# jcmgray/cotengra

Measured on AMD Instinct MI355X. Metric: contracted FLOP/s (whole node), Sycamore n53 m20 sliced amplitude, higher is better.
Workload: dtype complex64; 1 GPU; Sycamore n53 m20 amplitude, sliced tree, one slice per step per GPU; network=examples/benchmarks/sycamore_n53_m20_s0_e0_pABCDCDAB.json, tree=sycamore_m20_native.json, width_log2=32, parallelism=slice-parallel x1, 1 RCCL reduce, arithmetic=fp16x2 stem pairs and long tiled steps + fp32 MFMA

## Files before the change

cotengra_amd/csrc/ctg_common.h:

```cpp
#pragma once

#include <hip/hip_runtime.h>
#include <cstdlib>
#include <type_traits>
#include <stdint.h>

namespace ctg {

inline bool env_on(const char* name) {
    const char* v = getenv(name);
    return v != nullptr && v[0] != '\0' && !(v[0] == '0' && v[1] == '\0');
}
inline int env_state(const char* name) { return getenv(name) == nullptr ? -1 : (env_on(name) ? 1 : 0); }

inline hipError_t lds_opt_in(const void* kern, int bytes, unsigned long long* done) {
    int dev = 0;
    hipError_t e = hipGetDevice(&dev);
    if (e != hipSuccess) return e;
    const unsigned long long bit = 1ull << (dev & 63);
    if (__atomic_load_n(done, __ATOMIC_ACQUIRE) & bit) return hipSuccess;
    e = hipFuncSetAttribute(kern, hipFuncAttributeMaxDynamicSharedMemorySize, bytes);
    if (e != hipSuccess) {
        (void)hipGetLastError();
        return e;
// ... 353 lines not shown
inline hipError_t for_each_z(const StepArgs& p, F launch_one) {
    if (p.nz <= 1) return launch_one(p);
    for (int z = 0; z < p.nz; ++z) {
        StepArgs q = p;
        q.z0 = p.z0 + z;
        q.nz = 1;
        const hipError_t e = launch_one(q);
        if (e != hipSuccess) return e;
    }
    return hipSuccess;
}

template <typename F>
inline hipError_t for_each_z_chunk(const StepArgs& p, int64_t fit, F launch_chunk) {
    if (fit < 1) fit = 1;
    for (int64_t z = 0; z < p.nz; z += fit) {
        StepArgs q = p;
        q.z0 = p.z0 + (int32_t)z;
        q.nz = (int32_t)(p.nz - z < fit ? p.nz - z : fit);
        const hipError_t e = launch_chunk(q);
        if (e != hipSuccess) return e;
    }
    return hipSuccess;
}


hipError_t launch_pair_valu(int dtype, const StepArgs& p, void* scratch, int64_t scratch_bytes,
                            hipStream_t stream);
struct ValuGroupItem {
    StepArgs p;
    int64_t col_tiles, n_tiles;
    int32_t tn_shift;
    uint32_t block_begin, n_blocks;
};
constexpr int64_t kValuGroupMaxTiles = 4096;
bool valu_thread_per_output(const StepArgs& p);
void pair_valu_name(int dtype, const StepArgs& p, int64_t scratch_bytes, char* buf, size_t n);
uint32_t valu_group_fill(const StepArgs& p, ValuGroupItem* it, uint32_t block_begin);
hipError_t launch_pair_valu_group(int dtype, const ValuGroupItem* d_items, int n_items, uint32_t blocks,
                                  int nz, hipStream_t stream);
hipError_t launch_pair_mfma(int dtype, const StepArgs& p, const MfmaHints& h, void* scratch,
                            int64_t scratch_bytes, hipStream_t stream);
constexpr int64_t kPickKredMinK = 1 << 15, kPickKredMaxM = 512;
inline bool pick_route_kred(int64_t M, int64_t K) { return K >= kPickKredMinK && M <= kPickKredMaxM; }
hipError_t launch_pair_pick(int dtype, const StepArgs& p, int vec, void* scratch, int64_t scratch_bytes,
                            hipStream_t stream);
void pair_pick_name(int dtype, const StepArgs& p, int vec, int64_t scratch_bytes, char* buf, size_t n);
constexpr int64_t kPickRowsMfmaMinRowLo = 32, kPickRowsMfmaMinN = 8, kPickRowsMfmaMinK = 8;
inline bool pick_rows_route_mfma(int64_t row_lo, int64_t K, int64_t N, int dtype) {
    return dtype == 2 && row_lo >= kPickRowsMfmaMinRowLo && N >= kPickRowsMfmaMinN && K >= kPickRowsMfmaMinK;
}
hipError_t launch_pair_pick_rows(int dtype, const StepArgs& p, int vec, int b_fixed, hipStream_t stream);
void pair_pick_rows_name(int dtype, const StepArgs& p, int vec, int b_fixed, char* buf, size_t n);
struct FastGroupItem {
    StepArgs p;
    MfmaHints h;
    int64_t tiles_m, tiles_n;
    uint32_t block_begin, n_blocks;
};
constexpr int64_t kFastGroupMaxTiles = 128;
int fast_group_key(const StepArgs& p, const MfmaHints& h);
uint32_t fast_group_fill(const StepArgs& p, const MfmaHints& h, FastGroupItem* it, uint32_t block_begin);
hipError_t launch_pair_mfma_fast_group(int key, const FastGroupItem* d_items, int n_items, uint32_t blocks,
                                       int nz, hipStream_t stream);
bool rowwise_ok(const StepArgs& p);
void pair_mfma_c64_name(const StepArgs& p, const MfmaHints& h, int64_t scratch_bytes, char* buf, size_t n);
int64_t fast_lane_table_bytes();
hipError_t launch_fast_lane_consts(const StepArgs& p, const MfmaHints& h, void* out, hipStream_t stream);
hipError_t launch_pair_mfma_c128(const StepArgs& p, int flags, hipStream_t stream);
void pair_mfma_c128_name(const StepArgs& p, char* buf, size_t n);
hipError_t launch_pair_mfma_real(int dtype, const StepArgs& p, int flags, hipStream_t stream);
void pair_mfma_real_name(int dtype, const StepArgs& p, int flags, char* buf, size_t n);
bool stem2_supported(const StemArgs& p);
bool stem3_supported(const StemArgs& p);
hipError_t launch_stem2(const StemArgs& p, hipStream_t stream);
void stem2_kernel_name(const StemArgs& p, char* buf, size_t n);
bool stem2h_supported(const StemArgs& p);
bool stem2h_uses_h2(const StemArgs& p);
bool stem2_uses_bf3(const StemArgs& p);
hipError_t launch_stem2h(const StemArgs& p, hipStream_t stream);
void stem2h_kernel_name(const StemArgs& p, char* buf, size_t n);
int stem2_last_paired();
int stem2h_last_paired();

hipError_t launch_single(int dtype, const StepArgs& p, hipStream_t stream);
bool pair_bf16x3_on(const StepArgs& p);
hipError_t launch_accum(int dtype, const StepArgs& p, const StripState* st, void* wide, const double* inscale, int leaf,
                        hipStream_t stream);
struct AccumGroupItem {
    StepArgs p;
    void* wide;
    int32_t leaf;
    uint32_t block_begin, n_blocks;
};
constexpr int64_t kAccumGroupMaxBlocks = 1 << 16;
uint32_t accum_group_fill(const StepArgs& p, void* wide, int leaf, AccumGroupItem* it, uint32_t block_begin);
hipError_t launch_accum_group(int dtype, const AccumGroupItem* d_items, int n_items, uint32_t blocks, int nz,
                              const double* inscale, hipStream_t stream);
hipError_t launch_prescale_inputs(int dtype, void* inputs, const int64_t* offs, const int64_t* sizes, int64_t n_inputs,
                                  int* shift_total, double* inscale, hipStream_t stream);
hipError_t launch_narrow(int dtype, void* result, const void* wide, int64_t n, hipStream_t stream);
hipError_t launch_widen(int dtype, void* wide, const void* result, int64_t n, hipStream_t stream);

hipError_t launch_maxabs(int dtype, const void* x, int64_t n, double* fac, hipStream_t stream);
hipError_t launch_strip_prepare(const double* fac, const int32_t* counted, int64_t n_steps,
                                int64_t root_step, int check_zero, StripState* st, const double* inscale, hipStream_t stream);
hipError_t launch_rescale(int dtype, void* result, int64_t n, const StripState* st, hipStream_t stream);

struct SliceMeta {
    int64_t n_leaves;
    int64_t n_sliced;
    const int64_t* sizes;
    const int64_t* fixed;
    const int64_t* strides;
    double* fac;
    const int32_t* fac_zero;
    int64_t n_fac;
    float* smax;
    const int32_t* smax_zero;
    int64_t n_smax;
};
hipError_t launch_prologue(const SliceMeta& m, int64_t* state, int64_t* soff, int64_t sid,
                           hipStream_t stream, int nz = 1, int64_t stride = 1, const int64_t* ids = nullptr);
hipError_t launch_set_state(int64_t* state, int64_t next, int64_t stride, hipStream_t stream);

}
```

cotengra_amd/csrc/ctg_exec_state.h:

```cpp
#pragma once

#include <string>
#include <vector>

#include "../../include/ctg_hip.h"
#include "ctg_common.h"
#include "ctg_lds.h"

struct ctg_plan {
    int dtype = 0;
    int64_t n_inputs = 0;
    std::vector<int64_t> input_sizes, input_offsets;
    int64_t inputs_elems = 0, arena_elems = 0, result_elems = 0;
    int64_t n_steps = 0;
    std::vector<int64_t> steps;
    std::vector<int64_t> tables;
    int64_t n_sliced = 0;
    std::vector<int64_t> slice_sizes, slice_fixed, slice_strides;
    std::vector<int64_t> slice_group;
    bool has_groups = false;
    int64_t nslices = 1;
    std::vector<int64_t> max_soff;
};

struct ctg_exec {
    const ctg_plan* plan = nullptr;
    int device = 0;
    hipStream_t stream = nullptr;
    char* d_inputs = nullptr;
    char* d_arena = nullptr;
    char* d_result = nullptr;
    bool owns_result = false;
    char* d_wide = nullptr;
    int64_t* d_in_tab = nullptr;
    double* d_inscale = nullptr;
    int64_t* d_tables = nullptr;
    int64_t* d_misc = nullptr;
    int64_t* d_state = nullptr;
    int64_t* d_zero = nullptr;
    int64_t* d_soff = nullptr;
    void* d_scratch = nullptr;
    ctg::SliceMeta meta{};
    std::vector<ctg::StepArgs> args;
    std::vector<ctg::StemArgs> stem_args;
    int stem_bf16x3 = 1;
    int stem_arith = 2;
    float* d_stem_max = nullptr;
    int32_t* d_smax_zero = nullptr;
    float* smax_slot(int bank, int64_t s, int64_t z) const {
        return d_stem_max + (((int64_t)bank * plan_steps + s) * (batch > 1 ? batch : 1) + z) * ctg::kMaxSub;
    }
    ctg::SliceMeta meta_resetting(int which) const {
        ctg::SliceMeta m = meta;
        if (m.smax) m.smax_zero = d_smax_zero + (int64_t)which * m.n_smax;
        return m;
    }
    int64_t plan_steps = 0;
    std::vector<char> rec_wanted;
    std::vector<char> wave_member;
    std::vector<char> stem_paired_ran;
    std::vector<char> stem_h2_ran;
    std::vector<ctg::MfmaHints> hints;
    std::vector<ctg::MfmaHints> hints_b;
    uint16_t* d_ord_b = nullptr;
    char* d_lane_b = nullptr;
    uint16_t* d_ord = nullptr;
    char* d_lane = nullptr;
    int batch = 1;
    int group_d = 0;
    int64_t* d_batch_ids = nullptr;
    int64_t* h_ids = nullptr;
    size_t h_ids_cap = 0;
    hipEvent_t ev_ids = nullptr;
    int batch_nominal = 1;
    int64_t scratch_total = 0;
    struct Issue {
        int64_t step;
        int cls;
        int32_t item0, n;
        uint32_t blocks;
        bool shared = false;
    };
    std::vector<Issue> issue;
    std::vector<Issue> issue_reuse;
    std::vector<int32_t> lds_comp_of;
    int lds_first[2] = {0, 0}, lds_count[2] = {0, 0}, lds_bytes[2] = {0, 0};
    std::vector<std::vector<ctg::LdsForm>> lds_forms;
    ctg::LdsCompDev* d_lds_comps = nullptr;
    char* d_lds_blob = nullptr;
    ctg::ValuGroupItem* d_group_items = nullptr;
    ctg::AccumGroupItem* d_accum_items = nullptr;
    std::vector<char> accum_member;
    ctg::FastGroupItem* d_fast_items = nullptr;
    std::vector<hipEvent_t> events;
    hipStream_t gstream = nullptr;
    hipGraphExec_t gexec = nullptr;
    hipEvent_t ev_in = nullptr, ev_out = nullptr;
    bool warm = false;
    bool soff_static = false;
    bool graph_off = false;
    int strip = 0, check_zero = 0;
    double* d_fac = nullptr;
    int32_t* d_counted = nullptr;
    int32_t* d_fac_zero = nullptr;
    std::vector<char> invariant;
    bool invariants_ready = false;
    std::vector<char> grouped;
    int64_t group_key = -1;
    ctg::StripState* d_strip = nullptr;
    int64_t root_step = -1;
    void* d_sample_blocks = nullptr;
    void* d_sample_io = nullptr;
    int64_t sample_blocks_bytes = 0, sample_io_bytes = 0;
    double sample_last[4] = {0, 0, 0, 0};
    float sample_pass_ms[2] = {0, 0};
    bool sample_last_valid = false;
    hipEvent_t sample_ev[3] = {nullptr, nullptr, nullptr};
    void* d_range = nullptr;
    int64_t range_bytes = 0;
    void* d_reduce = nullptr;
    int64_t reduce_bytes = 0;
};


inline int64_t ctg_item_size(int dtype) {
    static const int64_t k[4] = {4, 8, 8, 16};
    return k[dtype];
}

extern "C" __attribute__((visibility("hidden"))) void ctg_set_error_(const char* msg);

namespace ctg {
hipError_t launch_maxabs_f32(const void* base, const int64_t* soff, int64_t z, int64_t zs, int64_t zstride, int64_t n,
                             float* out, hipStream_t stream, int nz = 1, int out_zs = 0);
}

namespace ctg {
constexpr int64_t kRangeMaxBlocks = 2048;
constexpr int64_t kRangeMaxComponents = 1ll << 40;
int64_t range_blocks(int64_t n);
int64_t range_partial_bytes(int64_t blocks);
hipError_t launch_range_hist(const void* x, int64_t n, void* partials, int64_t blocks, int64_t* row, double* sumsq,
// ... 24 lines not shown
```

cotengra_amd/csrc/ctg_runtime.hip:

```cpp
#include <algorithm>
#include <cstdarg>
#include <cmath>
#include <cstdio>
#include <cstdlib>
#include <cstring>
#include <string>
#include <vector>

#include "ctg_exec_state.h"

using namespace ctg;

namespace {

thread_local std::string g_err;

int fail(int code, const char* fmt, ...) {
    char buf[1024];
    va_list ap;
    va_start(ap, fmt);
    vsnprintf(buf, sizeof(buf), fmt, ap);
    va_end(ap);
    g_err = buf;
    return code;
// ... 1046 lines not shown
}

static bool tiled16_step(const ctg_exec* e, int64_t s) {
    const ctg_plan* p = e->plan;
    const int64_t* r = &p->steps[s * STEP_WORDS];
    if (r[W_KIND] != KIND_PAIR || r[W_KERNEL] != KERNEL_MFMA || p->dtype != CTG_C64) return false;
    const MfmaHints& h = e->hints[s];
    return !h.stream && h.fast && h.bf3 && e->stem_arith != 0 && !e->strip && e->d_stem_max != nullptr &&
           pair_bf16x3_on(e->args[s]);
}

static bool stem_step_h2(const ctg_exec* e, int64_t s, bool recorded) {
    return e->stem_arith == 2 && !e->strip && e->d_stem_max != nullptr && (recorded || env_on("CTG_STEM_H2_ALL")) &&
           stem2h_uses_h2(e->stem_args[s]) && env_state("CTG_STEM_H2") != 0;
}
static bool pair_step_h2(const ctg_exec* e, bool single) {
    return e->stem_arith == 2 && single && env_state("CTG_PAIR_H2") != 0;
}

static bool pair_records(const ctg_exec* e, int64_t s) {
    const ctg_plan* p = e->plan;
    const int64_t* r = &p->steps[s * STEP_WORDS];
    if (r[W_KIND] != KIND_PAIR || r[W_KERNEL] != KERNEL_MFMA || p->dtype != CTG_C64) return false;
    if (e->stem_arith == 0 || e->strip || e->d_stem_max == nullptr || e->grouped[s]) return false;
    const MfmaHints& h = e->hints[s];
    if (tiled16_step(e, s)) return h.splitk <= 1 && e->args[s].zqA <= 1 && e->args[s].zqB <= 1;
    if (e->stem_arith != 2 || e->wave_member[s] || !e->rec_wanted[s]) return false;
    return h.stream == 1 || (!h.stream && h.fast && !h.bf3 && h.splitk <= 1);
}

int launch_step(ctg_exec* e, int64_t s, hipStream_t stream) {
    const ctg_plan* p = e->plan;
    const int64_t* r = &p->steps[s * STEP_WORDS];
    hipError_t err = hipSuccess;
    if (!e->d_scratch && step_needs_scratch(e, s)) {
        const int rc = ensure_scratch(e);
        if (rc != CTG_OK) return rc;
    }
    switch (r[W_KIND]) {
        case KIND_SINGLE: err = launch_single(p->dtype, e->args[s], stream); break;
        case KIND_ACCUM:
            if (e->strip) {
                err = launch_strip_prepare(e->d_fac, e->d_counted, p->n_steps, e->root_step,
                                           e->check_zero, e->d_strip, e->d_inscale, stream);
                if (err == hipSuccess)
                    err = launch_rescale(p->dtype, e->d_result, p->result_elems, e->d_strip, stream);
                if (err == hipSuccess && e->d_wide)
                    err = launch_rescale(p->dtype + 1, e->d_wide, p->result_elems, e->d_strip, stream);
                if (err == hipSuccess) err = launch_accum(p->dtype, e->args[s], e->d_strip, wide_of_step(e, s), nullptr, -1, stream);
            } else {
                err = launch_accum(p->dtype, e->args[s], nullptr, wide_of_step(e, s), e->d_inscale, accum_leaf(p, s), stream);
            }
            break;
        case KIND_STEM2: {
            const int nz = e->args[s].nz;
            const bool rec = e->stem_arith != 0 && !e->strip && e->d_stem_max != nullptr;
            const int64_t prod = r[W_A_PROD];
            const bool prod_rec = prod >= 0 && prod < p->n_steps && e->stem_h2_ran[prod];
            const bool h2 = stem_step_h2(e, s, prod_rec);
            const bool records = h2 || (rec && stem2_uses_bf3(e->stem_args[s]));
            e->stem_h2_ran[s] = records ? 1 : 0;
            if (env_on("CTG_STEM_DEBUG"))
                fprintf(stderr, "stem step %lld: arith %d rec %d prod %lld prod_rec %d uses_h2 %d uses_bf3 %d -> h2 %d records %d\n",
                        (long long)s, e->stem_arith, (int)rec, (long long)prod, (int)prod_rec, (int)stem2h_uses_h2(e->stem_args[s]),
                        (int)stem2_uses_bf3(e->stem_args[s]), (int)h2, (int)records);
            for (int z = 0; z < nz && err == hipSuccess; ++z) {
                StemArgs q = e->stem_args[s];
                q.z0 = e->args[s].z0 + z;
                q.nz = 1;
                const int64_t zc = (e->invariant[s] || e->grouped[s]) ? 0 : q.z0;
                const int64_t za = (prod_rec && (e->invariant[prod] || e->grouped[prod])) ? 0 : q.z0;
                q.amax = h2 ? e->smax_slot(0, prod_rec ? prod : 0, za) : nullptr;
                q.cmax = records ? e->smax_slot(0, s, zc) : nullptr;
                if (h2 && !prod_rec) {
                    float* slot = e->smax_slot(1, s, q.z0);
                    err = hipMemsetAsync(slot, 0, sizeof(float) * kMaxSub, stream);
                    if (err == hipSuccess)
                        err = r[W_A_LEAF] >= 0 ? launch_maxabs_f32(q.A, nullptr, 0, 0, 0, q.a_elems, slot, stream)
                                               : launch_maxabs_f32(q.A, q.soffA, q.z0, q.zsA, q.zA, q.a_elems, slot, stream);
                    q.amax = slot;
                }
                if (err == hipSuccess) err = h2 ? launch_stem2h(q, stream) : launch_stem2(q, stream);
                if (err == hipSuccess) e->stem_paired_ran[s] = (char)(h2 ? stem2h_last_paired() : stem2_last_paired());
            }
            break;
        }
        case KIND_PAIR:
            if (r[W_KERNEL] == KERNEL_MFMA && p->dtype == CTG_C128)
                err = launch_pair_mfma_c128(e->args[s], e->hints[s].vecA , stream);
            else if (r[W_KERNEL] == KERNEL_MFMA && p->dtype != CTG_C64)
                err = launch_pair_mfma_real(p->dtype, e->args[s], e->hints[s].vecA, stream);
            else if (r[W_KERNEL] == KERNEL_MFMA) {
                const MfmaHints& h0 = (e->args[s].nz > 1 && !e->hints_b.empty()) ? e->hints_b[s] : e->hints[s];
                const bool tiled16 = tiled16_step(e, s) && !h0.stream && h0.fast && h0.bf3;
                if (tiled16) {
                    MfmaHints h = h0;
                    const StepArgs& a = e->args[s];
                    const bool single = h0.splitk <= 1 && a.zqA <= 1 && a.zqB <= 1 && !e->grouped[s] &&
                                        a.z0 + a.nz <= std::max(e->batch, 1);
                    const bool h2 = pair_step_h2(e, single);
                    h.h2 = h2 ? 1 : 0;
                    h.cmax = single ? e->smax_slot(0, s, 0) : nullptr;
                    h.cmax_zs = e->invariant[s] ? 0 : 1;
                    e->stem_h2_ran[s] = single ? 1 : 0;
                    for (int side = 0; side < 2 && h2 && err == hipSuccess; ++side) {
                        const int64_t prod = r[side == 0 ? W_A_PROD : W_B_PROD];
                        const float* mx = nullptr;
                        int zs = 1;
                        if (prod >= 0 && prod < p->n_steps && e->stem_h2_ran[prod] && !e->grouped[prod]) {
                            mx = e->smax_slot(0, prod, 0);
                            zs = e->invariant[prod] ? 0 : 1;
                        } else if (r[side == 0 ? W_A_LEAF : W_B_LEAF] >= 0) {
                            float* slot = e->smax_slot(1 + side, s, 0);
                            err = hipMemsetAsync(slot, 0, sizeof(float) * kMaxSub, stream);
                            if (err == hipSuccess)
                                err = launch_maxabs_f32(side == 0 ? a.A : a.B, nullptr, 0, 0, 0, r[side == 0 ? W_A_SIZE : W_B_SIZE], slot, stream);
                            mx = slot;
                            zs = 0;
                        } else {
                            float* slot = e->smax_slot(1 + side, s, 0);
                            float* at = slot + (int64_t)a.z0 * kMaxSub;
                            err = hipMemsetAsync(at, 0, sizeof(float) * kMaxSub * (size_t)a.nz, stream);
                            if (err == hipSuccess)
                                err = side == 0 ? launch_maxabs_f32(a.A, a.soffA, a.z0, a.zsA, a.zA, r[W_A_SIZE], at, stream, a.nz, kMaxSub)
                                                : launch_maxabs_f32(a.B, a.soffB, a.z0, a.zsB, a.zB, r[W_B_SIZE], at, stream, a.nz, kMaxSub);
                            mx = slot;
                        }
                        (side == 0 ? h.amax : h.bmax) = mx;
                        (side == 0 ? h.amax_zs : h.bmax_zs) = zs;
                    }
                    if (env_on("CTG_STEM_DEBUG"))
                        fprintf(stderr, "tiled step %lld: arith %d single %d -> h2 %d records %d (A prod %lld, B prod %lld)\n",
                                (long long)s, e->stem_arith, (int)single, (int)h2, (int)single, (long long)r[W_A_PROD],
                                (long long)r[W_B_PROD]);
                    if (err == hipSuccess) err = launch_pair_mfma(p->dtype, e->args[s], h, e->d_scratch, kScratchBytes, stream);
                } else {
                    const StepArgs& a = e->args[s];
                    const bool can = e->stem_arith == 2 && !e->strip && e->d_stem_max != nullptr && !e->grouped[s] &&
                                     !env_on("CTG_NO_PAIR_RECORD") &&
                                     !e->wave_member[s] && e->rec_wanted[s] && a.z0 + a.nz <= std::max(e->batch, 1) &&
                                     ((h0.stream == 1) || (!h0.stream && h0.fast && !h0.bf3 && h0.splitk <= 1));
                    if (!e->stem_h2_ran.empty()) e->stem_h2_ran[s] = can ? 1 : 0;
                    if (can) {
                        MfmaHints h = h0;
                        h.cmax = e->smax_slot(0, s, 0);
                        h.cmax_zs = e->invariant[s] ? 0 : 1;
                        err = launch_pair_mfma(p->dtype, a, h, e->d_scratch, kScratchBytes, stream);
                    } else {
                        err = launch_pair_mfma(p->dtype, a, h0, e->d_scratch, kScratchBytes, stream);
                    }
                }
            } else if (r[W_KERNEL] == KERNEL_PICK)
                err = launch_pair_pick(p->dtype, e->args[s], e->hints[s].vecA, e->d_scratch, kScratchBytes, stream);
            else if (r[W_KERNEL] == KERNEL_PICK_ROWS)
                err = launch_pair_pick_rows(p->dtype, e->args[s], e->hints[s].vecA, e->hints[s].fast, stream);
            else
                err = launch_pair_valu(p->dtype, e->args[s], e->d_scratch, kScratchBytes, stream);
            break;
    }
    if (err == hipSuccess && e->strip && (r[W_KIND] == KIND_PAIR || r[W_KIND] == KIND_STEM2)) {
        const char* c = (const char*)space_ptr(e, r[W_C_SPACE]) + r[W_C_OFF] * kItemSize[p->dtype];
        err = launch_maxabs(p->dtype, c, r[W_C_SIZE], e->d_fac + s, stream);
    }
    if (err != hipSuccess)
        return fail(CTG_E_HIP, "launch of step %lld failed: %s", (long long)s, hipGetErrorString(err));
    return CTG_OK;
// ... 529 lines not shown
        init[0] = 1.0;
        HIP_TRY_E(hipMalloc((void**)&e->d_inscale, init.size() * sizeof(double)));
        HIP_TRY_E(hipMemcpy(e->d_inscale, init.data(), init.size() * sizeof(double), hipMemcpyHostToDevice));
    }
    {
        bool sums = false;
        for (int64_t s = 0; s < p->n_steps; ++s) sums = sums || p->steps[s * STEP_WORDS + W_KIND] == KIND_ACCUM;
        sums = sums && p->nslices > 1;
        if (sums && (p->dtype == CTG_F32 || p->dtype == CTG_C64) && !env_on("CTG_NO_WIDE_SUM")) {
            HIP_TRY_E(hipMalloc((void**)&e->d_wide, p->result_elems * 2 * isz));
            HIP_TRY_E(hipMemsetAsync(e->d_wide, 0, p->result_elems * 2 * isz, e->stream));
        }
    }
    HIP_TRY_E(hipMalloc((void**)&e->d_tables, p->tables.size() * 8));
    e->scratch_total = kScratchBytes * std::min<int64_t>(std::max(e->batch, 1), 8);
    const int64_t n_leaves = p->n_inputs + 1;
    const int64_t misc_words = 3 + n_leaves * e->batch + 2 * p->n_sliced + n_leaves * p->n_sliced + e->batch;
    HIP_TRY_E(hipMalloc((void**)&e->d_misc, misc_words * 8));
    std::vector<int64_t> misc(misc_words, 0);
    int64_t* cur = e->d_misc;
    e->d_state = cur;
    cur += 2;
    e->d_zero = cur;
    cur += 1;
    e->d_soff = cur;
    cur += n_leaves * e->batch;
    int64_t* d_sizes = cur;
    cur += p->n_sliced;
    int64_t* d_fixed = cur;
    cur += p->n_sliced;
    int64_t* d_strides = cur;
    e->d_batch_ids = d_strides + n_leaves * p->n_sliced;
    for (int64_t j = 0; j < p->n_sliced; ++j) {
        misc[(d_sizes - e->d_misc) + j] = p->slice_sizes[j];
        misc[(d_fixed - e->d_misc) + j] = p->slice_fixed[j];
    }
    for (int64_t i = 0; i < n_leaves * p->n_sliced; ++i)
        misc[(d_strides - e->d_misc) + i] = p->slice_strides[i];
    misc[1] = 1;
    HIP_TRY_E(hipMemcpy(e->d_misc, misc.data(), misc_words * 8, hipMemcpyHostToDevice));
    HIP_TRY_E(hipMemcpy(e->d_tables, p->tables.data(), p->tables.size() * 8, hipMemcpyHostToDevice));
    HIP_TRY_E(hipMemsetAsync(e->d_inputs, 0, p->inputs_elems * isz, e->stream));
    HIP_TRY_E(hipMemsetAsync(e->d_result, 0, p->result_elems * isz, e->stream));
    e->meta = SliceMeta{n_leaves, p->n_sliced, d_sizes, d_fixed, d_strides, nullptr, nullptr, 0, nullptr, nullptr, 0};
    {
        std::vector<double> fac(p->n_steps + 1, 0.0);
        fac[p->n_steps] = 1.0;
        std::vector<int32_t> counted(std::max<int64_t>(p->n_steps, 1), 0);
        std::vector<int32_t> fac_zero(std::max<int64_t>(p->n_steps, 1), 0);
        e->invariant.assign(p->n_steps, 0);
        e->grouped.assign(p->n_steps, 0);
        for (int64_t st = 0; st < p->n_steps; ++st)
            e->grouped[st] = p->has_groups && p->steps[st * STEP_WORDS + W_INVARIANT] == 2 &&
                             p->steps[st * STEP_WORDS + W_KIND] != KIND_ACCUM;
        for (int64_t st = 0; st < p->n_steps; ++st) {
            const int64_t* r = &p->steps[st * STEP_WORDS];
            e->invariant[st] = r[W_INVARIANT] == 1 && r[W_KIND] != KIND_ACCUM;
            if (r[W_KIND] == KIND_PAIR || r[W_KIND] == KIND_STEM2) {
                counted[st] = 1;
                fac_zero[st] = e->invariant[st] ? 0 : 1;
                e->root_step = st;
            }
        }
        {
            bool stems = false;
            const int64_t nb = std::max<int64_t>(e->batch, 1);
            e->plan_steps = p->n_steps;
            const size_t bank = (size_t)(std::max<int64_t>(p->n_steps, 1) * nb * kMaxSub);
            std::vector<int32_t> sz(3 * bank, 0);
            for (int64_t st = 0; st < p->n_steps; ++st) {
                const int64_t* rs = &p->steps[st * STEP_WORDS];
                stems = stems || rs[W_KIND] == KIND_STEM2;
                const bool can = rs[W_KIND] == KIND_STEM2 || (rs[W_KIND] == KIND_PAIR && rs[W_KERNEL] == KERNEL_MFMA);
                if (!can) continue;
                for (int64_t z = 0; z < nb * kMaxSub; ++z) {
                    const size_t at = (size_t)(st * nb * kMaxSub + z);
                    sz[at] = e->invariant[st] ? 0 : 1;
                    sz[bank + at] = (e->invariant[st] || e->grouped[st]) ? 0 : 1;
                    sz[2 * bank + at] = 1;
                }
            }
            e->stem_h2_ran.assign(p->n_steps, 0);
            e->stem_paired_ran.assign(p->n_steps, 0);
            if (e->wave_member.size() != (size_t)p->n_steps) e->wave_member.assign(p->n_steps, 0);
            (void)stems;
            if (p->dtype == CTG_C64) {
                HIP_TRY_E(hipMalloc((void**)&e->d_stem_max, sz.size() * sizeof(float)));
                HIP_TRY_E(hipMemset(e->d_stem_max, 0, sz.size() * sizeof(float)));
                HIP_TRY_E(hipMalloc((void**)&e->d_smax_zero, sz.size() * sizeof(int32_t)));
                HIP_TRY_E(hipMemcpy(e->d_smax_zero, sz.data(), sz.size() * sizeof(int32_t), hipMemcpyHostToDevice));
                e->meta.smax = e->d_stem_max;
                e->meta.smax_zero = e->d_smax_zero;
                e->meta.n_smax = (int64_t)(sz.size() / 3);
            }
        }
        HIP_TRY_E(hipMalloc((void**)&e->d_fac_zero, fac_zero.size() * sizeof(int32_t)));
        HIP_TRY_E(hipMemcpy(e->d_fac_zero, fac_zero.data(), fac_zero.size() * sizeof(int32_t),
                            hipMemcpyHostToDevice));
        HIP_TRY_E(hipMalloc((void**)&e->d_fac, fac.size() * sizeof(double)));
        HIP_TRY_E(hipMalloc((void**)&e->d_counted, counted.size() * sizeof(int32_t)));
        HIP_TRY_E(hipMalloc((void**)&e->d_strip, sizeof(StripState)));
        HIP_TRY_E(hipMemcpy(e->d_fac, fac.data(), fac.size() * sizeof(double), hipMemcpyHostToDevice));
        HIP_TRY_E(hipMemcpy(e->d_counted, counted.data(), counted.size() * sizeof(int32_t),
                            hipMemcpyHostToDevice));
    }
    e->graph_off = !env_on("CTG_GRAPH");
    if (const char* v = getenv("CTG_STEM_ARITH")) {
        const std::string a(v);
        if (a == "fp32" || a == "0") e->stem_arith = 0;
        else if (a == "bf16x3" || a == "1") e->stem_arith = 1;
        else if (a == "fp16x2" || a == "2") e->stem_arith = 2;
        e->stem_bf16x3 = e->stem_arith ? 1 : 0;
    }
    resolve_args(e);
    {
        int rc = build_hints(e);
        if (rc == CTG_OK) rc = build_groups(e);
        for (int64_t st = 0; rc == CTG_OK && st < p->n_steps; ++st)
            if (step_needs_scratch(e, st)) {
                rc = ensure_scratch(e);
                break;
            }
        if (rc != CTG_OK) return bail(rc);
    }
    *out = e;
    return CTG_OK;
#undef HIP_TRY_E
}

int ctg_exec_set_stream(ctg_exec* e, void* stream) {
    if (!e) return fail(CTG_E_INVALID, "null argument");
    if ((hipStream_t)stream == e->stream) return CTG_OK;
    HIP_TRY(hipSetDevice(e->device));
    HIP_TRY(hipStreamSynchronize(e->stream));
    e->stream = (hipStream_t)stream;
    return CTG_OK;
}

int ctg_exec_upload_inputs_host(ctg_exec* e, const void* const* ptrs) {
    if (!e || !ptrs) return fail(CTG_E_INVALID, "null argument");
    HIP_TRY(hipSetDevice(e->device));
    const ctg_plan* p = e->plan;
    const int64_t isz = kItemSize[p->dtype];
    std::vector<char> staging((size_t)(p->inputs_elems * isz), 0);
    for (int64_t i = 0; i < p->n_inputs; ++i) {
        if (!ptrs[i]) return fail(CTG_E_INVALID, "input %lld is null", (long long)i);
        memcpy(staging.data() + p->input_offsets[i] * isz, ptrs[i], p->input_sizes[i] * isz);
    }
    HIP_TRY(hipStreamSynchronize(e->stream));
    HIP_TRY(hipMemcpy(e->d_inputs, staging.data(), staging.size(), hipMemcpyHostToDevice));
    if (e->d_inscale)
        HIP_TRY(launch_prescale_inputs(p->dtype, e->d_inputs, e->d_in_tab, e->d_in_tab + p->n_inputs, p->n_inputs,
                                       (int*)(e->d_inscale + 2), e->d_inscale, e->stream));
    e->invariants_ready = false;
    e->group_key = -1;
    return CTG_OK;
}

int ctg_exec_upload_inputs_device(ctg_exec* e, const void* const* ptrs) {
    if (!e || !ptrs) return fail(CTG_E_INVALID, "null argument");
    HIP_TRY(hipSetDevice(e->device));
    const ctg_plan* p = e->plan;
    const int64_t isz = kItemSize[p->dtype];
    for (int64_t i = 0; i < p->n_inputs; ++i) {
        if (!ptrs[i]) return fail(CTG_E_INVALID, "input %lld is null", (long long)i);
        HIP_TRY(hipMemcpyAsync(e->d_inputs + p->input_offsets[i] * isz, ptrs[i],
// ... 448 lines not shown
    bool lds_done[2] = {false, false};
    for (int64_t s = 0; s < p->n_steps; ++s) {
        if (e->invariant[s]) continue;
        if (!e->lds_comp_of.empty() && e->lds_comp_of[s] >= 0) {
            const int cls = e->grouped[s] ? 0 : 1;
            if (!lds_done[cls] && p->steps[s * STEP_WORDS + W_KIND] == KIND_PAIR) {
                lds_done[cls] = true;
                const ctg_exec::Issue q{s, -2, e->lds_first[cls], e->lds_count[cls], (uint32_t)e->lds_count[cls], cls == 0};
                const int rc = launch_issue(e, q, 1, e->stream);
                if (rc != CTG_OK) return rc;
            }
            continue;
        }
        {
            const int rc = launch_step(e, s, e->stream);
            if (rc != CTG_OK) return rc;
        }
        if (!audited(s)) continue;
        const int64_t* r = &p->steps[s * STEP_WORDS];
        const int rc = pass(e->d_arena, r[W_C_OFF], r[W_C_SIZE], p->arena_elems, p->n_inputs + s);
        if (rc != CTG_OK) return rc;
    }
    HIP_TRY(hipMemcpyAsync(rows, d_rows, (size_t)rows_bytes, hipMemcpyDeviceToHost, e->stream));
    HIP_TRY(hipMemcpyAsync(sumsq, d_sumsq, (size_t)(T * 8), hipMemcpyDeviceToHost, e->stream));
    HIP_TRY(hipStreamSynchronize(e->stream));
    return CTG_OK;
}

int ctg_exec_step_kernel(ctg_exec* e, int64_t step, char* buf, int64_t buflen) {
    if (!e || !buf || buflen < 1) return fail(CTG_E_INVALID, "null argument");
    const ctg_plan* p = e->plan;
    if (step < 0 || step >= p->n_steps) return fail(CTG_E_INVALID, "step out of range");
    const int64_t* r = &p->steps[step * STEP_WORDS];
    char name[128];
    if (!e->lds_comp_of.empty() && e->lds_comp_of[step] >= 0) {
        snprintf(name, sizeof(name), "lds_run_kernel[%d]", (int)e->lds_comp_of[step]);
    } else if (r[W_KIND] == KIND_SINGLE) {
        snprintf(name, sizeof(name), "single_kernel");
    } else if (r[W_KIND] == KIND_ACCUM) {
        snprintf(name, sizeof(name), (size_t)step < e->accum_member.size() && e->accum_member[step] ? "accum_group_kernel"
                                                                                                    : "accum_kernel");
    } else if (r[W_KIND] == KIND_STEM2) {
        const int64_t prod = r[W_A_PROD];
        const bool prod16 = prod >= 0 && prod < p->n_steps &&
                            ((p->steps[prod * STEP_WORDS + W_KIND] == KIND_STEM2 &&
                              (stem2_uses_bf3(e->stem_args[prod]) || stem2h_uses_h2(e->stem_args[prod]))) ||
                             pair_records(e, prod));
        if (stem_step_h2(e, step, prod16)) stem2h_kernel_name(e->stem_args[step], name, sizeof(name));
        else stem2_kernel_name(e->stem_args[step], name, sizeof(name));
    } else if (r[W_KERNEL] == KERNEL_MFMA && p->dtype == CTG_C128) {
        pair_mfma_c128_name(e->args[step], name, sizeof(name));
    } else if (r[W_KERNEL] == KERNEL_MFMA && p->dtype != CTG_C64) {
        pair_mfma_real_name(p->dtype, e->args[step], e->hints[step].vecA, name, sizeof(name));
    } else if (r[W_KERNEL] == KERNEL_MFMA) {
        MfmaHints h = e->hints[step];
        h.h2 = pair_step_h2(e, tiled16_step(e, step) && h.splitk <= 1 && !e->grouped[step] &&
                                   e->args[step].zqA <= 1 && e->args[step].zqB <= 1) ? 1 : 0;
        pair_mfma_c64_name(e->args[step], h, kScratchBytes, name, sizeof(name));
    } else if (r[W_KERNEL] == KERNEL_PICK) {
        pair_pick_name(p->dtype, e->args[step], e->hints[step].vecA, kScratchBytes, name, sizeof(name));
    } else if (r[W_KERNEL] == KERNEL_PICK_ROWS) {
        pair_pick_rows_name(p->dtype, e->args[step], e->hints[step].vecA, e->hints[step].fast, name, sizeof(name));
    } else {
        pair_valu_name(p->dtype, e->args[step], kScratchBytes, name, sizeof(name));
    }
    snprintf(buf, (size_t)buflen, "%s", name);
    return CTG_OK;
}

int ctg_plan_stem_pair16(ctg_plan* p, int64_t step, int* ok) {
    if (!p || !ok) return fail(CTG_E_INVALID, "null argument");
    if (step < 0 || step >= p->n_steps) return fail(CTG_E_INVALID, "step out of range");
    *ok = p->steps[step * STEP_WORDS + W_KIND] == KIND_STEM2 && stem_pair16_ok(p, step) ? 1 : 0;
    return CTG_OK;
}

int ctg_exec_step_paired_stores(ctg_exec* e, int64_t step, int* paired) {
    if (!e || !paired) return fail(CTG_E_INVALID, "null argument");
    if (step < 0 || step >= e->plan->n_steps) return fail(CTG_E_INVALID, "step out of range");
    *paired = (size_t)step < e->stem_paired_ran.size() && e->stem_paired_ran[step] ? 1 : 0;
    return CTG_OK;
}

int ctg_exec_step_stem_max(ctg_exec* e, int64_t step, int64_t z, float* mx) {
    if (!e || !mx) return fail(CTG_E_INVALID, "null argument");
    const ctg_plan* p = e->plan;
    if (step < 0 || step >= p->n_steps) return fail(CTG_E_INVALID, "step out of range");
    if (z < 0 || z >= (e->batch > 1 ? e->batch : 1)) return fail(CTG_E_INVALID, "slice of the batch out of range");
    if (e->d_stem_max == nullptr || (size_t)step >= e->stem_h2_ran.size() || !e->stem_h2_ran[step] ||
        p->steps[step * STEP_WORDS + W_KIND] != KIND_STEM2)
        return fail(CTG_E_INVALID, "step %lld has recorded no maximum", (long long)step);
    HIP_TRY(hipSetDevice(e->device));
    HIP_TRY(hipStreamSynchronize(e->stream));
    float rec[kMaxSub];
    HIP_TRY(hipMemcpy(rec, e->smax_slot(0, step, (e->invariant[step] || e->grouped[step]) ? 0 : z), sizeof(rec), hipMemcpyDeviceToHost));
    *mx = rec[0];
    for (int i = 1; i < kMaxSub; ++i) *mx = std::max(*mx, rec[i]);
    return CTG_OK;
}

int ctg_exec_sync(ctg_exec* e) {
    if (!e) return fail(CTG_E_INVALID, "null argument");
    HIP_TRY(hipSetDevice(e->device));
    HIP_TRY(hipStreamSynchronize(e->stream));
    return CTG_OK;
}

int ctg_exec_result_ptr(ctg_exec* e, void** dev_ptr) {
    if (!e || !dev_ptr) return fail(CTG_E_INVALID, "null argument");
    *dev_ptr = e->d_result;
    return CTG_OK;
}

int ctg_exec_download_result(ctg_exec* e, void* host_out) {
    if (!e || !host_out) return fail(CTG_E_INVALID, "null argument");
    HIP_TRY(hipSetDevice(e->device));
    HIP_TRY(hipStreamSynchronize(e->stream));
    HIP_TRY(hipMemcpy(host_out, e->d_result, e->plan->result_elems * kItemSize[e->plan->dtype],
                      hipMemcpyDeviceToHost));
    return CTG_OK;
}

int ctg_exec_download_arena(ctg_exec* e, int64_t offset, int64_t n, void* host_out) {
    if (!e || !host_out) return fail(CTG_E_INVALID, "null argument");
    if (offset < 0 || n < 0 || offset + n > e->plan->arena_elems)
        return fail(CTG_E_BOUNDS, "arena range out of bounds");
    const int64_t isz = kItemSize[e->plan->dtype];
    HIP_TRY(hipSetDevice(e->device));
    HIP_TRY(hipStreamSynchronize(e->stream));
    HIP_TRY(hipMemcpy(host_out, e->d_arena + offset * isz, n * isz, hipMemcpyDeviceToHost));
    return CTG_OK;
}

}
```

cotengra_amd/csrc/ctg_stem.hip:

```cpp
#include "ctg_stem_impl.h"

namespace ctg {
#ifdef CTG_STEM_DEV_ONE
#ifdef CTG_STEM_DEV_P16
template __global__ void stem2_kernel_p16<CTG_STEM_DEV_ONE>(StemArgs);
#else
template __global__ void stem2_kernel<CTG_STEM_DEV_ONE>(StemArgs);
#endif
#else
int stem2_last_paired() { return stem_last_paired; }
bool stem2_supported(const StemArgs& p) { return stem2_supported_shape(p); }
bool stem3_supported(const StemArgs& p) { return stem3_supported_shape(p); }
bool stem2_uses_bf3(const StemArgs& p) { return stem_uses_16bit(p); }
void stem2_kernel_name(const StemArgs& p, char* buf, size_t n) { stem_kernel_name<Bf16x3>(p, buf, n); }
hipError_t launch_stem2(const StemArgs& p, hipStream_t stream) { return launch_stem<Bf16x3>(p, stream); }
#endif
}

#ifndef CTG_STEM_DEV_ONE
extern "C" int ctg_stem_triple_instantiated(int p1, int pm, int p2, int rt1, int cs1, int nch, int itm, int it2, int vec) {
    return ctg::stem3_instantiated(p1 != 0, pm != 0, p2 != 0, rt1, cs1, nch, itm, it2, vec != 0) ? 1 : 0;
}
#endif
#ifdef CTG_STEM_TIMELINE
extern "C" int ctg_debug_stem_timeline(unsigned long long* out, int reset) { return ctg::stem_debug_timeline<ctg::Bf16x3>(out, reset); }
#endif
#ifdef CTG_STEM_BOUNDS
extern "C" int ctg_debug_stem_oob(unsigned long long out[2], int reset) { return ctg::stem_debug_oob<ctg::Bf16x3>(out, reset); }
#endif
```

cotengra_amd/csrc/ctg_stem_h2.hip:

```cpp
#include "ctg_stem_impl.h"

namespace ctg {
#ifdef CTG_STEM_DEV_ONE
#ifdef CTG_STEM_DEV_P16
template __global__ void stem2h_kernel_p16<CTG_STEM_DEV_ONE>(StemArgs);
#else
template __global__ void stem2h_kernel<CTG_STEM_DEV_ONE>(StemArgs);
#endif
#else
int stem2h_last_paired() { return stem_last_paired; }
bool stem2h_supported(const StemArgs& p) { return stem2_supported_shape(p); }
bool stem2h_uses_h2(const StemArgs& p) { return stem_uses_16bit(p); }
void stem2h_kernel_name(const StemArgs& p, char* buf, size_t n) { stem_kernel_name<Fp16x2>(p, buf, n); }
hipError_t launch_stem2h(const StemArgs& p, hipStream_t stream) { return launch_stem<Fp16x2>(p, stream); }
#endif
}

#ifdef CTG_STEM_TIMELINE
extern "C" int ctg_debug_stem_timeline_h2(unsigned long long* out, int reset) { return ctg::stem_debug_timeline<ctg::Fp16x2>(out, reset); }
#endif
#ifdef CTG_STEM_BOUNDS
extern "C" int ctg_debug_stem_oob_h2(unsigned long long out[2], int reset) { return ctg::stem_debug_oob<ctg::Fp16x2>(out, reset); }
#endif
```

cotengra_amd/csrc/ctg_stem_impl.h:

```cpp
#pragma once
#include "ctg_common.h"

#include <cstdio>
#include <cstdlib>
#include <type_traits>


namespace ctg {

typedef float f32x16 __attribute__((ext_vector_type(16)));
typedef float f32x4 __attribute__((ext_vector_type(4)));

#ifdef CTG_STEM_BOUNDS
template <class AR>
__device__ unsigned long long ctg_stem_oob[2];
#endif

#ifdef CTG_STEM_TIMELINE
#define CTG_TL_TILES 256
template <class AR>
__device__ unsigned long long ctg_stem_tl[8][CTG_TL_TILES][6];
template <class AR>
__device__ int ctg_stem_tl_on;
#endif
// ... 135 lines not shown
                                                  int N, int planes, int tid, bool vec, float scale) {
    const int ROW = bf3_row(K, STEP1);
    for (int e = tid; e < K * N; e += SW * 64) {
        const int k = e / N, n = e - k * N;
        int at;
        if (STEP1) {
            const int h = vec ? (k >> 1) & 1 : k & 1;
            const int slot = vec ? (((k & 15) >> 2) << 1) | (k & 1) : (k & 15) >> 1;
            at = (k >> 4) * 48 + h * 24 + slot;
        } else {
            at = (k >> 3) * 24 + (k & 7);
        }
        const c64 v = B[off[e]];
        const float vals[3] = {v.re * scale, v.im * scale, -v.im * scale};
#pragma unroll
        for (int pl = 0; pl < 3; ++pl) {
            if (pl >= planes) break;
            AR::store_limbs(Q + (pl * N + n) * ROW + at, vals[pl]);
        }
    }
}

template <class AR>
__device__ __forceinline__ int bf3_operand_exponent(const c64* __restrict__ B, const int64_t* off, int n_el, int tid,
                                                    float* red) {
    float mx = 0.f;
    for (int e = tid; e < n_el; e += SW * 64) {
        const c64 v = B[off[e]];
        mx = fmaxf(mx, fmaxf(fabsf(v.re), fabsf(v.im)));
    }
#pragma unroll
    for (int o = 32; o > 0; o >>= 1) mx = fmaxf(mx, __shfl_xor(mx, o));
    if ((tid & 63) == 0) red[tid >> 6] = mx;
    __syncthreads();
    mx = red[0];
#pragma unroll
    for (int w = 1; w < SW; ++w) mx = fmaxf(mx, red[w]);
    __syncthreads();
    return AR::operand_exponent(mx);
}
__device__ __forceinline__ int h2_exponent_of(float mx) {
    const int ex = (int)((__builtin_bit_cast(unsigned, mx) >> 23) & 255u) - 127;
    if (mx == 0.f || ex == 128 || ex == -127) return 0;
    const int e = ex - 13;
    return e < -126 ? -126 : (e > 126 ? 126 : e);
}
__device__ __forceinline__ float pow2f(int ex) {
    return __builtin_bit_cast(float, (unsigned)(ex + 127) << 23);
}

}

#ifdef CTG_STEM_TIMELINE
#define CTG_TL_STAMP(k)                                                                                   \
    do {                                                                                                  \
        if (blockIdx.x == 0 && lane == 0 && tl_n < CTG_TL_TILES && ctg_stem_tl_on<AR>)                    \
            ctg_stem_tl<AR>[wave][tl_n][k] = __builtin_readcyclecounter();                                \
        if ((k) == 5) ++tl_n;                                                                             \
    } while (0)
#else
#define CTG_TL_STAMP(k) do {} while (0)
#endif

template <typename T>
__device__ __forceinline__ void settle(T& v) {
    asm volatile("" : "+v"(v));
}

#ifndef CTG_STEM_WS_DEPTH
#define CTG_STEM_WS_DEPTH 2
#endif
#ifndef CTG_STEM_DEPTH
#define CTG_STEM_DEPTH 2
#endif
#ifndef CTG_STEM_GATHER_PORTIONS
#define CTG_STEM_GATHER_PORTIONS 1
#endif
#ifndef CTG_STEM_NT_STORES
#define CTG_STEM_NT_STORES 1
#endif
constexpr bool STEM_NT_STORES = CTG_STEM_NT_STORES != 0;
constexpr bool STEM_GATHER_PORTIONS = CTG_STEM_GATHER_PORTIONS != 0;
template <class AR, bool PACK1, bool PACK2, int RT1_, int CS1, int NCH, int IT2_, bool BR1, int K2Q, bool VEC, bool BF3,
          bool RI2, bool ONE, int ITM, bool PACKM, bool XM, bool LM, bool WS, bool P16 = false>
__device__ __forceinline__ void stem2_body(const StemArgs& p) {
    constexpr bool TRI = ITM > 0;
    static_assert(!P16 || (XM && !PACK2 && NCH > 0 && ((WS && IT2_ == 1) || (!WS && IT2_ == 2))),
                  "paired stores: a wave whose two items are the two column groups of a row tile");
    static_assert(!LM, "reserved (the limb intermediate was removed): kernel names stay 17 arguments long");
    static_assert(BF3 || !AR::fp16, "fp16 x 2: the 16-bit kernels only (its object has no fp32 products)");
    static_assert(!AR::fp16 || !TRI, "fp16 x 2: pairs and single steps");
    static_assert(!WS || (XM && !ONE && IT2_ > 0 && IT2_ <= 2 && (PACK1 || RT1_ == 1)), "specialised waves: a static 16-bit pair");
    constexpr int PW = WS ? 4 : SW;
    constexpr int RT1 = WS ? 2 * RT1_ : RT1_;
    constexpr int IT2 = WS ? 2 * IT2_ : IT2_;
    static_assert(!XM || (BF3 && !TRI && NCH > 0), "two-accumulator real part: bf16 x 3, static, no three-step tile");
    constexpr bool XM1 = XM && !PACK1 && !WS;
    constexpr bool XM2 = XM && !PACK2;
    static_assert(!TRI || (NCH > 0 && IT2 > 0 && !RI2 && !ONE && K2Q == 0), "three-step tile: static, X / Y form");
    static_assert(!ONE || (!PACK1 && !PACK2 && !RI2 && IT2 == 0 && K2Q == 0), "one step: >= 32 columns, nothing of step 2");
    static_assert(!PACK1 || CS1 == 1, "16 columns are one group");
    static_assert(!BR1 || NCH > 0, "B1 in registers needs the chunk count at compile time");
    static_assert(K2Q == 0 || PACK2 || IT2 == 1 || RI2, "B2 in registers: one column group per wave");
    static_assert(!RI2 || (!PACK2 && !BF3 && NCH > 0 && IT2 > 0), "row-interleaved step 2: fp32, >= 32 columns, static");
    constexpr bool SH1 = WS && CS1 > 1 && RT1 % CS1 == 0;
    constexpr int CG1 = SH1 ? CS1 : 1;
    constexpr int RR1 = RT1 / CG1;
    constexpr int RTW = SH1 ? PW : PW / CS1;
    constexpr bool STATIC = NCH > 0;
    extern __shared__ __attribute__((aligned(16))) char smem[];
    const int K1 = p.K1, N1 = p.N1, K2 = K2Q > 0 ? 4 * K2Q : p.K2, N2 = p.N2;
    const int LDB1 = K1 + 4, LDB2 = K2 + 4, LD2 = K2Q > 0 ? 4 * K2Q + 4 : p.ld2;
    const int PLANE = p.rows2 * LD2;
    const int KM = TRI ? p.KM : 0, NM = TRI ? p.NM : 0, LDM = TRI ? p.ldM : 0, LDBM = KM + 4;
    const int PLANEM = TRI ? p.rowsM * LDM : 0;
    const int PLANE1 = TRI ? PLANEM : PLANE;
    float* P1 = (float*)smem;
    float* PM = P1 + (PACK1 ? 3 : 2) * N1 * LDB1;
    float* P2 = PM + (TRI ? (PACKM ? 3 : 2) * NM * LDBM : 0);
    float* mid = P2 + (PACK2 ? 3 : 2) * N2 * LDB2;
    const int RP = 3 * LD2;
    auto ri_off = [&](int e) __attribute__((always_inline)) { return RI2 ? (e / LD2) * RP + e % LD2 : e; };
    int mid_floats = 2 * (PLANE > PLANEM ? PLANE : PLANEM);
    if constexpr (RI2) {
        mid_floats = 3 * PLANE;
        if constexpr (K2Q > 0) {
            mid = P2;
            const int p2f = 2 * N2 * LDB2;
            mid_floats = mid_floats > p2f ? mid_floats : p2f;
        }
    }
    const int ROW1 = bf3_row(K1, true), ROW2 = bf3_row(K2, false), ROWM = TRI ? bf3_row(KM, false) : 0;
    unsigned short* Q1 = (unsigned short*)smem;
    unsigned short* QM = Q1 + (PACK1 ? 3 : 2) * N1 * ROW1;
    unsigned short* Q2 = QM + (TRI ? (PACKM ? 3 : 2) * NM * ROWM : 0);
    if constexpr (BF3) mid = (float*)(Q2 + (PACK2 ? 3 : 2) * N2 * ROW2);
    int64_t* oc_s = (int64_t*)(mid + ((mid_floats + 1) & ~1));

    const int tid = threadIdx.x;
    const int lane = tid & 63;
    const int wave = __builtin_amdgcn_readfirstlane(tid >> 6);
    const int kk = lane >> 5;
    const int l31 = lane & 31;
    const bool producer = !WS || wave < PW;
    const int wave1 = WS ? (wave & (PW - 1)) : wave;
    const int wrt = SH1 ? wave1 : wave1 / CS1;
    const int wcol = SH1 ? 0 : (wave1 % CS1) * 32;

    const int64_t z = (int64_t)p.z0 + blockIdx.y;
    const c64* __restrict__ A = (const c64*)p.A + (sload64(p.soffA + z * p.zsA) + z * p.zA);
    const c64* __restrict__ B1 = (const c64*)p.B1 + (sload64(p.soffB1 + z * p.zsB1) + z * p.zB1);
    const c64* __restrict__ B2 = (const c64*)p.B2 + (sload64(p.soffB2 + z * p.zsB2) + z * p.zB2);
    float* __restrict__ C = (float*)((c64*)p.C + (sload64(p.soffC + z * p.zsC) + z * p.zC));
    const c64* __restrict__ BM = TRI ? (const c64*)p.BM + (sload64(p.soffBM + z * p.zsBM) + z * p.zBM) : nullptr;

    int bf3_ex = 0;
    float* const bf3_red = (float*)(oc_s + (ONE ? N1 : N2));
    float h2_sa = 1.f;
    int h2_exa = 0;
    if constexpr (AR::fp16) {
        h2_exa = p.amax != nullptr ? h2_exponent_of(read_max(p.amax)) : 0;
        h2_exa = __builtin_amdgcn_readfirstlane(h2_exa);
        h2_sa = pow2f(-h2_exa);
    }
    float h2_st = 1.f;
    float h2_vmax = 0.f;
    if constexpr (BF3) {
        const int ex1 = bf3_operand_exponent<AR>(B1, p.b1_off, K1 * N1, tid, bf3_red);
        const int ex2 = ONE ? 0 : bf3_operand_exponent<AR>(B2, p.b2_off, K2 * N2, tid, bf3_red);
        int exm = 0;
        if constexpr (TRI) {
            exm = bf3_operand_exponent<AR>(BM, p.bm_off, KM * NM, tid, bf3_red);
            load_b_planes_bf3<AR, false>(QM, BM, p.bm_off, KM, NM, PACKM ? 3 : 2, tid, false, pow2f(-exm));
        }
        bf3_ex = ex1 + ex2 + exm;
        load_b_planes_bf3<AR, true>(Q1, B1, p.b1_off, K1, N1, PACK1 ? 3 : 2, tid, VEC, pow2f(-ex1));
        if constexpr (!ONE) load_b_planes_bf3<AR, false>(Q2, B2, p.b2_off, K2, N2, PACK2 ? 3 : 2, tid, false, pow2f(-ex2));
    } else {
        load_b_planes<true>(P1, B1, p.b1_off, K1, N1, PACK1, tid, VEC);
        if constexpr (!ONE) load_b_planes<false>(P2, B2, p.b2_off, K2, N2, PACK2, tid);
        if constexpr (TRI) load_b_planes<false>(PM, BM, p.bm_off, KM, NM, PACKM, tid);
    }
    const int NOUT = ONE ? N1 : N2;
    for (int n = tid; n < NOUT; n += SW * 64) oc_s[n] = p.out_col[n];

    unsigned a_lane = (unsigned)(p.lane_a[lane] * 8);
    settle(a_lane);
    int64_t kj[8];
#pragma unroll
    for (int j = 0; j < 8; ++j) kj[j] = sload64(p.kj_a + j);
    const unsigned sgn = 0x80000000u;
    const float* b1p;
    const float* b1q;
    if (PACK1) {
        const int n = l31 & 15, h = l31 >> 4;
        b1p = P1 + ((h ? 1 : 0) * N1 + n) * LDB1 + kk * 8;
        b1q = P1 + ((h ? 0 : 2) * N1 + n) * LDB1 + kk * 8;
    } else {
        b1p = P1 + (wcol + l31) * LDB1 + kk * 8;
        b1q = P1 + (N1 + wcol + l31) * LDB1 + kk * 8;
    }
    const unsigned sgn2 = kk ? 0x80000000u : 0u;
    const unsigned short* q1p;
    const unsigned short* q1q;
    const unsigned short* q2x;
    const unsigned short* q2y = nullptr;
    {
        const int h16 = l31 >> 4;
        if (PACK1) {
            q1p = Q1 + ((h16 ? 1 : 0) * N1 + (l31 & 15)) * ROW1 + kk * 24;
            q1q = Q1 + ((h16 ? 0 : 2) * N1 + (l31 & 15)) * ROW1 + kk * 24;
        } else {
            q1p = Q1 + (wcol + l31) * ROW1 + kk * 24;
            q1q = Q1 + (N1 + wcol + l31) * ROW1 + kk * 24;
        }
        if (PACK2) {
            const int plane = kk == 0 ? (h16 ? 1 : 0) : (h16 ? 0 : 2);
            q2x = Q2 + (plane * N2 + (l31 & 15)) * ROW2;
        } else {
            q2x = Q2 + ((kk ? 1 : 0) * N2 + l31) * ROW2;
            q2y = Q2 + ((kk ? 0 : 1) * N2 + l31) * ROW2;
        }
    }
    const float* b2x;
    const float* b2y = nullptr;
    if (PACK2) {
        const int n = l31 & 15, h = l31 >> 4;
        const int plane = kk == 0 ? (h ? 1 : 0) : (h ? 0 : 2);
        b2x = P2 + (plane * N2 + n) * LDB2;
    } else {
        b2x = P2 + ((kk ? 1 : 0) * N2 + l31) * LDB2;
        b2y = P2 + ((kk ? 0 : 1) * N2 + l31) * LDB2;
    }
    int mid_lane[CG1];
#pragma unroll
    for (int cg = 0; cg < CG1; ++cg) {
        mid_lane[cg] = 0;
        if constexpr (!ONE) {
            if (PACK1) mid_lane[cg] = ri_off((int)p.mid_col[l31 & 15]) + (l31 >> 4) * (RI2 ? LD2 : PLANE1) + ri_off((int)p.mid_row[4 * kk]);
            else mid_lane[cg] = ri_off((int)p.mid_col[wcol + 32 * cg + l31]) + ri_off((int)p.mid_row[4 * kk]);
        }
        settle(mid_lane[cg]);
    }
    int mid_o[4];
#pragma unroll
    for (int b = 0; b < 4; ++b) mid_o[b] = ONE ? 0 : ri_off((int)sload64(p.mid_row + (b < 2 ? 1 << b : 2 << b)));
    int mid_rt[RT1];
    int64_t one_rt[RT1];
#pragma unroll
    for (int m = 0; m < RT1; ++m) {
        mid_rt[m] = ONE ? 0 : __builtin_amdgcn_readfirstlane(ri_off((int)sload64(p.mid_row + 32 * (wrt + RTW * (m / CG1)))));
        one_rt[m] = ONE ? sload64(p.out_row + 32 * (wrt + RTW * (m / CG1))) : 0;
    }
    const int64_t one_col = ONE ? p.out_col[wcol + l31] : 0;
    auto mid_t = [&](int t) __attribute__((always_inline)) {
        return ((t & 1) ? mid_o[0] : 0) + ((t & 2) ? mid_o[1] : 0) + ((t & 4) ? mid_o[2] : 0) + ((t & 8) ? mid_o[3] : 0);
    };
    int64_t out_lane = p.out_row[RI2 ? 2 * kk : 4 * kk];
    if (PACK2) out_lane += (l31 >> 4) ? p.out_row[1] : 0;
    settle(out_lane);
    int64_t out_o[4];
#pragma unroll
    for (int b = 0; b < 4; ++b) out_o[b] = sload64(p.out_row + (RI2 ? (b == 0 ? 1 : 2 << b) : (b < 2 ? 1 << b : 2 << b)));
    auto out_t = [&](int t) __attribute__((always_inline)) {
        return ((t & 1) ? out_o[0] : 0) + ((t & 2) ? out_o[1] : 0) + ((t & 4) ? out_o[2] : 0) + ((t & 8) ? out_o[3] : 0);
    };
    const int n_rtM = TRI ? p.rowsM >> 5 : 1;
    const unsigned short* qmx[TRI ? ITM : 1];
    const unsigned short* qmy[TRI ? ITM : 1];
    const float* bmx[TRI ? ITM : 1];
    const float* bmy[TRI ? ITM : 1];
    int m2_lane[TRI ? ITM : 1], m2_rt[TRI ? ITM : 1], am_row[TRI ? ITM : 1];
    int m2_o[4] = {0, 0, 0, 0};
    if constexpr (TRI) {
        const int h16 = l31 >> 4;
#pragma unroll
        for (int i = 0; i < ITM; ++i) {
            const int item = wave + SW * i;
            const int cg = item / n_rtM, rtm = item - cg * n_rtM;
            am_row[i] = (rtm * 32 + l31) * LDM;
            if (PACKM) {
                const int plane = kk == 0 ? (h16 ? 1 : 0) : (h16 ? 0 : 2);
                qmx[i] = QM + (plane * NM + (l31 & 15)) * ROWM;
                qmy[i] = nullptr;
                bmx[i] = PM + (plane * NM + (l31 & 15)) * LDBM;
                bmy[i] = nullptr;
                m2_lane[i] = (int)p.mid2_col[l31 & 15] + h16 * PLANE + (int)p.mid2_row[4 * kk];
            } else {
                qmx[i] = QM + ((kk ? 1 : 0) * NM + cg * 32 + l31) * ROWM;
                qmy[i] = QM + ((kk ? 0 : 1) * NM + cg * 32 + l31) * ROWM;
                bmx[i] = PM + ((kk ? 1 : 0) * NM + cg * 32 + l31) * LDBM;
                bmy[i] = PM + ((kk ? 0 : 1) * NM + cg * 32 + l31) * LDBM;
                m2_lane[i] = (int)p.mid2_col[cg * 32 + l31] + (int)p.mid2_row[4 * kk];
            }
            settle(m2_lane[i]);
            m2_rt[i] = __builtin_amdgcn_readfirstlane((int)sload64(p.mid2_row + 32 * rtm));
        }
#pragma unroll
        for (int b = 0; b < 4; ++b) m2_o[b] = (int)sload64(p.mid2_row + (b < 2 ? 1 << b : 2 << b));
    }
    auto m2_t = [&](int t) __attribute__((always_inline)) {
        return ((t & 1) ? m2_o[0] : 0) + ((t & 2) ? m2_o[1] : 0) + ((t & 4) ? m2_o[2] : 0) + ((t & 8) ? m2_o[3] : 0);
    };
    const int ri_par = l31 & 1;
    const int ri_plane = (ri_par == kk ? 0 : (ri_par ? 1 : 2)) * LD2;
    const int ri_cg = RI2 ? wave % p.ng2 : 0;
    const int ri_rt0 = RI2 ? wave / p.ng2 : 0;
    const int ri_rts = RI2 ? SW / p.ng2 : 0;
    const float* ri_b = P2 + (kk * N2 + ri_cg * 32 + l31) * LDB2;

    float alpha = 1.f, alpha2 = 1.f;
    {
        int e1 = bf3_ex < -126 ? -126 : (bf3_ex > 126 ? 126 : bf3_ex);
        int e2 = bf3_ex - e1;
        e2 = e2 < -126 ? -126 : (e2 > 126 ? 126 : e2);
        if (p.facA != nullptr) {
            const double f = (*p.facA) * (*p.facB1) * (*p.facB2) * (TRI ? *p.facBM : 1.0);
            alpha = (f == 0.0 && p.check_zero) ? 0.f : (float)(1.0 / f * (BF3 ? exp2((double)e1) : 1.0));
        } else if (BF3 && bf3_ex != 0) {
            alpha = pow2f(e1);
        }
        if (BF3 && e2 != 0) alpha2 = pow2f(e2);
    }
    const int h2_e0 = bf3_ex + h2_exa;
    auto h2_set_alpha = [&](int et) __attribute__((always_inline)) {
        const int E = h2_e0 + et;
        const int e1 = E < -126 ? -126 : (E > 126 ? 126 : E);
        int e2 = E - e1;
        e2 = e2 < -126 ? -126 : (e2 > 126 ? 126 : e2);
        alpha = pow2f(e1);
        alpha2 = pow2f(e2);
    };
    if constexpr (AR::fp16) h2_set_alpha(0);
    const bool scaled = AR::fp16 ? true : __builtin_amdgcn_readfirstlane(alpha != 1.f || alpha2 != 1.f);
    __syncthreads();

    f32x4 b1r[BR1 && !BF3 ? NCH * 2 : 1][2];
    f32x4 b2r[K2Q > 0 && !BF3 ? K2Q : 1][PACK2 ? 1 : 2];
    bf16x8 b1r3[CG1][BR1 && BF3 ? NCH : 1][3][2];
    const int q1cg = 32 * ROW1;
    if constexpr (BR1 && BF3) {
#pragma unroll
        for (int cg = 0; cg < CG1; ++cg)
#pragma unroll
            for (int c = 0; c < NCH; ++c)
#pragma unroll
                for (int q = 0; q < 3; ++q) {
                    b1r3[cg][c][q][0] = *(const bf16x8*)(q1p + cg * q1cg + c * 48 + q * 8);
                    b1r3[cg][c][q][1] = *(const bf16x8*)(q1q + cg * q1cg + c * 48 + q * 8);
                }
    }
    if constexpr (BR1 && !BF3) {
#pragma unroll
        for (int q = 0; q < NCH * 2; ++q) {
            b1r[q][0] = *(const f32x4*)(b1p + (q >> 1) * 16 + (q & 1) * 4);
            b1r[q][1] = *(const f32x4*)(b1q + (q >> 1) * 16 + (q & 1) * 4);
        }
    }
    if constexpr (K2Q > 0 && RI2) {
#pragma unroll
        for (int q = 0; q < K2Q; ++q) b2r[q][0] = *(const f32x4*)(ri_b + 4 * q);
    }
    if constexpr (K2Q > 0 && !BF3 && !RI2) {
        const int cg0 = PACK2 ? 0 : wave / (p.rows2 >> 5);
#pragma unroll
        for (int q = 0; q < K2Q; ++q) {
            b2r[q][0] = *(const f32x4*)(b2x + cg0 * 32 * LDB2 + 4 * q);
            if (!PACK2) {
                b2r[q][1] = *(const f32x4*)(b2y + cg0 * 32 * LDB2 + 4 * q);
#pragma unroll
                for (int t = 0; t < 4; ++t) b2r[q][0][t] = flip(b2r[q][0][t], sgn2);
            }
        }
    }
    const int nch = STATIC ? NCH : (K1 >> 4);
    const int n_rt2 = p.rows2 >> 5;
    const int n_items = n_rt2 * p.ng2;
    const int64_t n_tiles = p.n_tiles;
    const int64_t tile0 = blockIdx.x, tile_step = gridDim.x;
    const int64_t my_tiles = (n_tiles - tile0 + tile_step - 1) / tile_step;
    const int64_t last_tile = tile0 + (my_tiles - 1) * tile_step;

    constexpr int GD = WS ? CTG_STEM_WS_DEPTH : ((NCH > 0 && CTG_STEM_DEPTH == 4 && ((RT1 * NCH) & 1) == 0) ? 4 : 2);
    c64 regs[GD][8];
    int64_t ig = tile0;
    int im = 0, ic = 0;
    int64_t pend0 = 0, pend1 = 0, pend2 = 0, pend3 = 0;
    bool pend_live = false;
    auto prep = [&](auto always_tag) __attribute__((always_inline)) {
        constexpr bool ALWAYS = decltype(always_tag)::value;
        pend_live = ALWAYS || ig < n_tiles;
        if (pend_live) {
            const int64_t g = ALWAYS ? (ig < last_tile ? ig : last_tile) : ig;
            const int64_t gh = g >> p.g_lo_shift, gl = g & (p.g_lo - 1);
            pend0 = sload64(p.gA_hi + uniform64(gh));
            pend1 = sload64(p.gA_lo + uniform64(gl));
            pend2 = sload64(p.rt_a + (wrt + RTW * im));
            pend3 = sload64(p.chunk_a + ic);
            if (++ic == nch) {
                ic = 0;
                if (++im == RR1) {
                    im = 0;
                    ig += tile_step;
                }
            }
        }
    };
    auto fire2 = [&](c64 (&r)[8], int q, int64_t base, auto always_tag) __attribute__((always_inline)) {
        if (decltype(always_tag)::value || pend_live) {
            if constexpr (XM) {
                typedef const __attribute__((address_space(1))) char* gptr;
                uint64_t u0 = (uint64_t)A + ((uint64_t)(base + kj[2 * q]) << 3);
                uint64_t u1 = (uint64_t)A + ((uint64_t)(base + kj[2 * q + 1]) << 3);
                asm volatile("" : "+s"(u0), "+s"(u1));
                settle(a_lane);
                const unsigned al = a_lane;
                if (VEC) {
                    const f32x4 v = *(const __attribute__((address_space(1))) f32x4*)((gptr)u0 + al);
                    r[2 * q] = c64{v[0], v[1]};
                    r[2 * q + 1] = c64{v[2], v[3]};
                } else {
                    typedef float f32x2 __attribute__((ext_vector_type(2)));
                    const f32x2 v0 = *(const __attribute__((address_space(1))) f32x2*)((gptr)u0 + al);
                    const f32x2 v1 = *(const __attribute__((address_space(1))) f32x2*)((gptr)u1 + al);
                    r[2 * q] = c64{v0[0], v0[1]};
                    r[2 * q + 1] = c64{v1[0], v1[1]};
                }
                return;
            }
            const char* sb = (const char*)(A + (base + kj[2 * q]));
#ifdef CTG_STEM_BOUNDS
            {
                const uint64_t lim = (uint64_t)p.a_elems * 8;
                const uint64_t o0 = (uint64_t)(sb + a_lane - (const char*)A);
                const uint64_t o1 = VEC ? o0 + 8 : (uint64_t)((const char*)(A + (base + kj[2 * q + 1])) + a_lane - (const char*)A);
                if (o0 + 8 > lim || o1 + 8 > lim) {
                    atomicAdd(&ctg_stem_oob<AR>[0], 1ull);
                    r[2 * q] = r[2 * q + 1] = c64{0.f, 0.f};
                    return;
                }
            }
#endif
            if (VEC) {
                const f32x4 v = *(const f32x4*)(sb + a_lane);
                r[2 * q] = c64{v[0], v[1]};
                r[2 * q + 1] = c64{v[2], v[3]};
            } else {
                const char* sb1 = (const char*)(A + (base + kj[2 * q + 1]));
                const float2 v0 = *(const float2*)(sb + a_lane);
                const float2 v1 = *(const float2*)(sb1 + a_lane);
                r[2 * q] = c64{v0.x, v0.y};
                r[2 * q + 1] = c64{v1.x, v1.y};
            }
        }
    };
    auto issue = [&](c64 (&r)[8], auto always_tag) __attribute__((always_inline)) {
        prep(always_tag);
        const int64_t base = pend0 + pend1 + pend2 + pend3;
#pragma unroll
        for (int q = 0; q < 4; ++q) fire2(r, q, base, always_tag);
    };

#ifdef CTG_STEM_TIMELINE
    int tl_n = 0;
#endif
    f32x16 ax[RT1], ay[RT1];
    f32x16 axm[XM1 ? RT1 : 1];
    constexpr int NST = PACK2 ? 8 : 16;
    float2 pv[RI2 ? 1 : NST];
    float2 pw[P16 ? NST : 1];
    float* pdst = C;
    constexpr int NSET = RI2 ? (IT2 > 1 ? 2 : 1) : 1;
    f32x16 cr[NSET][2];
    auto store2 = [&](float* q, float2 v) __attribute__((always_inline)) {
#ifdef CTG_STEM_BOUNDS
        if ((uint64_t)((char*)q - (char*)C) + 8 > (uint64_t)p.c_elems * 8) {
            atomicAdd(&ctg_stem_oob<AR>[1], 1ull);
            return;
        }
#endif
        if constexpr (STEM_NT_STORES) {
            typedef float f32x2 __attribute__((ext_vector_type(2)));
            __builtin_nontemporal_store(f32x2{v.x, v.y}, (f32x2*)q);
        } else {
            *(float2*)q = v;
        }
    };
    auto store4 = [&](float* q, float2 v, float2 w) __attribute__((always_inline)) {
#ifdef CTG_STEM_BOUNDS
        if ((uint64_t)((char*)q - (char*)C) + 16 > (uint64_t)p.c_elems * 8) {
            atomicAdd(&ctg_stem_oob<AR>[1], 1ull);
            return;
        }
#endif
        if constexpr (STEM_NT_STORES) __builtin_nontemporal_store(f32x4{v.x, v.y, w.x, w.y}, (f32x4*)q);
        else *(f32x4*)q = f32x4{v.x, v.y, w.x, w.y};
    };
    auto drain = [&](int lo, int hi, auto set_tag, auto scaled_tag) __attribute__((always_inline)) {
        constexpr int SET = decltype(set_tag)::value < NSET ? decltype(set_tag)::value : 0;
#pragma unroll
        for (int i = lo; i < hi; ++i) {
            if constexpr (P16) {
                store4(pdst + 2 * out_t(i), pv[i], pw[i]);
            } else if constexpr (RI2) {
                float2 v;
                v.x = cr[SET][i >> 3][2 * (i & 7)];
                v.y = cr[SET][i >> 3][2 * (i & 7) + 1];
                if constexpr (decltype(scaled_tag)::value) {
                    v.x = v.x * alpha * alpha2;
                    v.y = v.y * alpha * alpha2;
                }
                store2(pdst + 2 * out_t(i), v);
            } else {
                store2(pdst + 2 * out_t(PACK2 ? 2 * i : i), pv[i]);
            }
        }
    };
    auto consume = [&](c64 (&r)[8], int m, int ch, auto always_tag, auto drain_tag, auto scaled_tag)
                       __attribute__((always_inline)) {
        constexpr bool DRAIN = decltype(drain_tag)::value >= 0;
        const int64_t base = pend0 + pend1 + pend2 + pend3;
        if constexpr (BF3) {
            float re[8], im[8];
#pragma unroll
            for (int j = 0; j < 8; ++j) {
                re[j] = r[j].re;
                im[j] = r[j].im;
            }
            bf16x8 r3[3], i3[3], n3[3], bp3[CG1][3], bq3[CG1][3];
            AR::split(re, r3, h2_sa);
            AR::split(im, i3, h2_sa);
            __builtin_amdgcn_sched_barrier(0);
            constexpr bool GP = STEM_GATHER_PORTIONS && decltype(always_tag)::value;
            if constexpr (!GP) {
#pragma unroll
                for (int q = 0; q < 4; ++q) fire2(r, q, base, always_tag);
            }
#pragma unroll
            for (int q = 0; q < 3; ++q) {
                if (!PACK1 && !XM1) n3[q] = __builtin_bit_cast(bf16x8, __builtin_bit_cast(u32x4, i3[q]) ^ 0x80008000u);
#pragma unroll
                for (int cg = 0; cg < CG1; ++cg) {
                    if constexpr (BR1) {
                        bp3[cg][q] = b1r3[cg][ch][q][0];
                        bq3[cg][q] = b1r3[cg][ch][q][1];
                    } else {
                        bp3[cg][q] = *(const bf16x8*)(q1p + cg * q1cg + ch * 48 + q * 8);
                        bq3[cg][q] = *(const bf16x8*)(q1q + cg * q1cg + ch * 48 + q * 8);
                    }
                }
            }
            __builtin_amdgcn_sched_barrier(0);
            const bool fresh = XM && STATIC && ch == 0;
            f32x16 zero16;
#pragma unroll
            for (int u = 0; u < 16; ++u) zero16[u] = 0.f;
#pragma unroll
            for (int t = 0; t < 6; t += AR::t_step(t)) {
                const int ta = bf3_ta(t), tb = bf3_tb(t);
                if constexpr (GP) {
                    constexpr int P = AR::products;
                    const int i = AR::t_index(t);
#pragma unroll
                    for (int q = (4 * i + P - 1) / P; q < (4 * (i + 1) + P - 1) / P; ++q) fire2(r, q, base, always_tag);
                }
                if (PACK1) {
                    ax[m] = AR::mfma(r3[ta], bp3[0][tb], (fresh && t == 0) ? zero16 : ax[m]);
                    ax[m] = AR::mfma(i3[ta], bq3[0][tb], ax[m]);
                } else if constexpr (XM1) {
                    ax[m] = AR::mfma(r3[ta], bp3[0][tb], (fresh && t == 0) ? zero16 : ax[m]);
                    ay[m] = AR::mfma(r3[ta], bq3[0][tb], (fresh && t == 0) ? zero16 : ay[m]);
                    axm[m] = AR::mfma(i3[ta], bq3[0][tb], (fresh && t == 0) ? zero16 : axm[m]);
                    ay[m] = AR::mfma(i3[ta], bp3[0][tb], ay[m]);
                } else {
#pragma unroll
                    for (int cg = 0; cg < CG1; ++cg) {
                        const int u = m * CG1 + cg;
                        ax[u] = AR::mfma(r3[ta], bp3[cg][tb], (fresh && t == 0) ? zero16 : ax[u]);
                        ay[u] = AR::mfma(r3[ta], bq3[cg][tb], (fresh && t == 0) ? zero16 : ay[u]);
                    }
#pragma unroll
                    for (int cg = 0; cg < CG1; ++cg) {
                        const int u = m * CG1 + cg;
                        ax[u] = AR::mfma(n3[ta], bq3[cg][tb], ax[u]);
                        ay[u] = AR::mfma(i3[ta], bp3[cg][tb], ay[u]);
                    }
                }
                __builtin_amdgcn_sched_barrier(0);
                if constexpr (DRAIN)
                    drain(AR::t_index(t) * NST / AR::products, (AR::t_index(t) + 1) * NST / AR::products, drain_tag, scaled_tag);
            }
            __builtin_amdgcn_sched_barrier(0);
            prep(always_tag);
            __builtin_amdgcn_sched_barrier(0);
            return;
        }
        f32x4 bp[2], bq[2];
        if constexpr (BR1) {
            bp[0] = b1r[ch * 2][0];
            bp[1] = b1r[ch * 2 + 1][0];
            bq[0] = b1r[ch * 2][1];
            bq[1] = b1r[ch * 2 + 1][1];
        } else {
            bp[0] = *(const f32x4*)(b1p + ch * 16);
            bq[0] = *(const f32x4*)(b1q + ch * 16);
            bp[1] = *(const f32x4*)(b1p + ch * 16 + 4);
            bq[1] = *(const f32x4*)(b1q + ch * 16 + 4);
        }
#pragma unroll
        for (int j = 0; j < 8; ++j) {
            const float re = r[j].re, im = r[j].im;
            const float p_ = bp[j >> 2][j & 3], q_ = bq[j >> 2][j & 3];
            __builtin_amdgcn_sched_barrier(0);
            if (PACK1) {
                ax[m] = mfma(re, p_, ax[m]);
                ax[m] = mfma(im, q_, ax[m]);
            } else {
                ax[m] = mfma(re, p_, ax[m]);
                ay[m] = mfma(re, q_, ay[m]);
                ax[m] = mfma(flip(im, sgn), q_, ax[m]);
                ay[m] = mfma(im, p_, ay[m]);
            }
            __builtin_amdgcn_sched_barrier(0);
            if (j & 1) fire2(r, j >> 1, base, always_tag);
            if constexpr (DRAIN) drain(j * NST / 8, (j + 1) * NST / 8, drain_tag, scaled_tag);
        }
        __builtin_amdgcn_sched_barrier(0);
        prep(always_tag);
        __builtin_amdgcn_sched_barrier(0);
    };
    auto zero_acc = [&](int m) __attribute__((always_inline)) {
        if constexpr (XM && STATIC) return;
#pragma unroll
        for (int t = 0; t < 16; ++t) {
            ax[m][t] = 0.f;
            if (!PACK1) ay[m][t] = 0.f;
            if constexpr (XM1) axm[m][t] = 0.f;
        }
    };
// ... 321 lines not shown
            const int col = P16 ? 64 * cg0 + 2 * l31 + G : cg * 32 + l31;
            const unsigned short* bR = Q2 + col * ROW2 + kk * 24;
            if constexpr (G == 1 && !P16) drain(0, NST, std::integral_constant<int, 0>{}, scaled_tag);
            if constexpr (G == 0) load_a(AK[0], 0);
            load_b(BF[0], bR, 0);
            static_for<0, NC>([&](auto ci) __attribute__((always_inline)) {
                constexpr int CH = decltype(ci)::value;
                if constexpr (CH + 1 < NC) {
                    if constexpr (G == 0) load_a(AK[CH + 1], CH + 1);
                    load_b(BF[(CH + 1) & 1], bR, CH + 1);
                }
                mul(AK[CH], BF[CH & 1], CH == 0);
            });
            emit(col, std::integral_constant<bool, (P16 && G == 1)>{});
        });
    };
    f32x16 mx[TRI ? ITM : 1], my[TRI ? ITM : 1];
    auto item_mid = [&](auto ii) __attribute__((always_inline)) {
        constexpr int I = decltype(ii)::value;
        f32x16 cx, cy;
#pragma unroll
        for (int t = 0; t < 16; ++t) {
            cx[t] = 0.f;
            cy[t] = 0.f;
        }
        const float* a_base = mid + kk * PLANEM + am_row[I];
        if constexpr (BF3) {
            for (int kb = 0; kb < (KM >> 3); ++kb) {
                const f32x4 lo = *(const f32x4*)(a_base + 8 * kb), hi = *(const f32x4*)(a_base + 8 * kb + 4);
                const float a8[8] = {lo[0], lo[1], lo[2], lo[3], hi[0], hi[1], hi[2], hi[3]};
                bf16x8 a3[3], ax3[3], bx3[3], by3[3];
                AR::split(a8, a3);
#pragma unroll
                for (int q = 0; q < 3; ++q) {
                    ax3[q] = PACKM ? a3[q]
                                   : __builtin_bit_cast(bf16x8, __builtin_bit_cast(u32x4, a3[q]) ^ (sgn2 | (sgn2 >> 16)));
                    bx3[q] = *(const bf16x8*)(qmx[I] + kb * 24 + q * 8);
                    if (!PACKM) by3[q] = *(const bf16x8*)(qmy[I] + kb * 24 + q * 8);
                }
#pragma unroll
                for (int t = 0; t < 6; t += AR::t_step(t)) {
                    cx = AR::mfma(ax3[bf3_ta(t)], bx3[bf3_tb(t)], cx);
                    if (!PACKM) cy = AR::mfma(a3[bf3_ta(t)], by3[bf3_tb(t)], cy);
                }
            }
        } else {
            const int nq = KM >> 2;
            f32x4 af[2], bx[2], by[2];
            af[0] = *(const f32x4*)(a_base);
            bx[0] = *(const f32x4*)(bmx[I]);
            if (!PACKM) by[0] = *(const f32x4*)(bmy[I]);
            for (int kq = 0; kq < nq; kq += 2) {
#pragma unroll
                for (int h = 0; h < 2; ++h) {
                    const int nx = (kq + h + 1 < nq ? kq + h + 1 : nq - 1) * 4;
                    af[(h + 1) & 1] = *(const f32x4*)(a_base + nx);
                    bx[(h + 1) & 1] = *(const f32x4*)(bmx[I] + nx);
                    if (!PACKM) by[(h + 1) & 1] = *(const f32x4*)(bmy[I] + nx);
                    __builtin_amdgcn_sched_barrier(0);
#pragma unroll
                    for (int t = 0; t < 4; ++t) {
                        if (PACKM) {
                            cx = mfma(af[h][t], bx[h][t], cx);
                        } else {
                            cx = mfma(flip(af[h][t], sgn2), bx[h][t], cx);
                            cy = mfma(af[h][t], by[h][t], cy);
                        }
                    }
                    __builtin_amdgcn_sched_barrier(0);
                }
            }
        }
        mx[I] = cx;
        my[I] = cy;
    };
    auto scatter_mid = [&](auto ii) __attribute__((always_inline)) {
        constexpr int I = decltype(ii)::value;
        float* dst = mid + (m2_lane[I] + m2_rt[I]);
#pragma unroll
        for (int t = 0; t < 16; ++t) {
            dst[m2_t(t)] = mx[I][t];
            if (!PACKM) dst[PLANE + m2_t(t)] = my[I][t];
        }
    };
    auto emit_one = [&](int m, int64_t c_tile, auto scaled_tag) __attribute__((always_inline)) {
        constexpr bool SC = decltype(scaled_tag)::value;
#pragma unroll
        for (int t = 0; t < 16; ++t) {
            float2 v;
            const float xr = XM1 ? ax[m][t] - axm[m][t] : ax[m][t];
            v.x = SC ? xr * alpha * alpha2 : xr;
            v.y = SC ? ay[m][t] * alpha * alpha2 : ay[m][t];
            if constexpr (BF3) h2_vmax = fmaxf(h2_vmax, fmaxf(fabsf(v.x), fabsf(v.y)));
            pv[RI2 ? 0 : t] = v;
        }
        pdst = C + 2 * (c_tile + one_rt[m] + out_lane + one_col);
    };
    int h2_par = 0;
    auto h2_publish = [&]() __attribute__((always_inline)) {
        if constexpr (AR::fp16 && !ONE) {
            float mx = 0.f;
#pragma unroll
            for (int m = 0; m < RT1; ++m)
#pragma unroll
                for (int t = 0; t < 16; ++t) {
                    const float xr = XM1 ? ax[m][t] - axm[m][t] : ax[m][t];
                    mx = fmaxf(mx, fabsf(xr));
                    if (!PACK1) mx = fmaxf(mx, fabsf(ay[m][t]));
                }
#pragma unroll
            for (int o = 32; o > 0; o >>= 1) mx = fmaxf(mx, __shfl_xor(mx, o));
            if (lane == 0) bf3_red[h2_par * 8 + wave1] = mx;
            if constexpr (WS) h2_par ^= 1;
        }
    };
    auto h2_consume = [&]() __attribute__((always_inline)) {
        if constexpr (AR::fp16 && !ONE) {
            float mx = bf3_red[h2_par * 8];
#pragma unroll
            for (int w = 1; w < PW; ++w) mx = fmaxf(mx, bf3_red[h2_par * 8 + w]);
            const int et = __builtin_amdgcn_readfirstlane(h2_exponent_of(mx));
            h2_st = pow2f(-et);
            h2_set_alpha(et);
            h2_par ^= 1;
        }
    };
    auto tile_c = [&](int64_t g) __attribute__((always_inline)) -> int64_t {
        const int64_t gh = g >> p.g_lo_shift, gl = g & (p.g_lo - 1);
        return sload64(p.gC_hi + uniform64(gh)) + sload64(p.gC_lo + uniform64(gl));
    };

    auto run = [&](auto scaled_tag) __attribute__((always_inline)) {
    if constexpr (WS) {
        constexpr int NT = RR1 * NCH;
        constexpr int U = (NT % GD == 0) ? 1 : ((2 * NT) % GD == 0 ? 2 : 4);
        static_assert((U * NT) % GD == 0, "a pass of U tiles returns to gather set 0");
        auto step1 = [&](auto slot0_tag) __attribute__((always_inline)) {
            constexpr int SLOT0 = decltype(slot0_tag)::value;
            static_for<0, RR1>([&](auto mi) __attribute__((always_inline)) {
                constexpr int M = decltype(mi)::value;
                static_for<0, NCH>([&](auto ci) __attribute__((always_inline)) {
                    constexpr int CH = decltype(ci)::value;
                    consume(regs[(SLOT0 + M * NCH + CH) & (GD - 1)], M, CH, std::true_type{}, std::integral_constant<int, -1>{}, scaled_tag);
                });
            });
        };
        auto step2 = [&](int64_t gc) __attribute__((always_inline)) {
            const int64_t c_tile = tile_c(gc);
            int64_t c_rows[IT2];
            if constexpr (IT2 == 2 && XM2) {
                if (P16 || n_rt2 <= PW) {
                    const int nc = K2 >> 4;
                    if (P16 || nc == 4) {
                        item2k(std::integral_constant<int, 4>{}, wave1, item_row(wave1, c_tile), scaled_tag);
                        return;
                    }
                    if (nc == 2) {
                        item2k(std::integral_constant<int, 2>{}, wave1, item_row(wave1, c_tile), scaled_tag);
                        return;
                    }
                }
            }
            static_for<0, IT2>([&](auto ii) __attribute__((always_inline)) {
                c_rows[decltype(ii)::value] = item_row(wave1 + PW * decltype(ii)::value, c_tile);
            });
            static_for<0, IT2>([&](auto ii) __attribute__((always_inline)) {
                constexpr int I = decltype(ii)::value;
                item2(wave1 + PW * I, c_rows[I], scaled_tag, std::integral_constant<bool, (I > 0)>{}, std::true_type{});
            });
        };
        if (producer) {
            static_for<0, GD>([&](auto gi) __attribute__((always_inline)) { issue(regs[decltype(gi)::value], std::true_type{}); });
            prep(std::true_type{});
            step1(std::integral_constant<int, 0>{});
            for (int64_t t = 0; t < my_tiles; t += U) {
                static_for<0, U>([&](auto ui) __attribute__((always_inline)) {
                    constexpr int UI = decltype(ui)::value;
                    if (t + UI < my_tiles) {
                        h2_publish();
                        __syncthreads();
                        scatter();
                        __syncthreads();
                        if (t + UI + 1 < my_tiles) step1(std::integral_constant<int, ((UI + 1) * NT) & (GD - 1)>{});
                    }
                });
            }
        } else {
            for (int64_t t = 0; t < my_tiles; ++t) {
                __syncthreads();
                if (t > 0) drain(0, NST, std::integral_constant<int, 0>{}, scaled_tag);
                __syncthreads();
                h2_consume();
                step2(tile0 + t * tile_step);
            }
            drain(0, NST, std::integral_constant<int, 0>{}, scaled_tag);
        }
    } else if constexpr (STATIC) {
        constexpr int NT = RT1 * NCH;
        constexpr int U = (NT % GD) ? 2 : 1;
        static_assert((U * NT) % GD == 0, "a pass of U tiles returns to gather set 0");
        constexpr int LASTSET = RI2 ? ((IT2 > 0 ? IT2 - 1 : 0) & (NSET - 1)) : 0;
        static_for<0, GD>([&](auto gi) __attribute__((always_inline)) { issue(regs[decltype(gi)::value], std::true_type{}); });
        prep(std::true_type{});
        int64_t g = tile0;
        auto tile = [&](auto slot0_tag, auto first_tag) __attribute__((always_inline)) {
            constexpr int SLOT0 = decltype(slot0_tag)::value;
            constexpr bool FIRST = decltype(first_tag)::value;
            if constexpr (ONE) {
                const int64_t c_tile = tile_c(g);
                static_for<0, RT1>([&](auto mi) __attribute__((always_inline)) {
                    constexpr int M = decltype(mi)::value;
                    zero_acc(M);
                    static_for<0, NCH>([&](auto ci) __attribute__((always_inline)) {
                        constexpr int CH = decltype(ci)::value;
                        consume(regs[(SLOT0 + M * NCH + CH) & (GD - 1)], M, CH, std::true_type{},
                                std::integral_constant<int, (CH == 0 && !(FIRST && M == 0)) ? 0 : -1>{}, scaled_tag);
                    });
                    emit_one(M, c_tile, scaled_tag);
                });
                g += tile_step;
                return;
            }
            CTG_TL_STAMP(0);
            static_for<0, RT1>([&](auto mi) __attribute__((always_inline)) {
                constexpr int M = decltype(mi)::value;
                zero_acc(M);
                static_for<0, NCH>([&](auto ci) __attribute__((always_inline)) {
                    constexpr int CH = decltype(ci)::value;
                    consume(regs[(SLOT0 + M * NCH + CH) & (GD - 1)], M, CH, std::true_type{},
                            std::integral_constant<int, (!FIRST && M == 0 && CH == 0) ? LASTSET : -1>{}, scaled_tag);
                });
            });
            CTG_TL_STAMP(1);
            h2_publish();
            __syncthreads();
            CTG_TL_STAMP(2);
            scatter();
            CTG_TL_STAMP(3);
            const int64_t c_tile = tile_c(g);
            int64_t c_rows[IT2 > 0 ? IT2 : 1];
            static_for<0, IT2>([&](auto ii) __attribute__((always_inline)) {
                constexpr int I = decltype(ii)::value;
                if constexpr (RI2) {
                    int64_t c_row = c_tile + sload64(p.out_row + 32 * (ri_rt0 + ri_rts * I));
                    asm volatile("" : "+s"(c_row));
                    c_rows[I] = c_row;
                } else {
                    c_rows[I] = item_row(wave + SW * I, c_tile);
                }
            });
            __syncthreads();
            h2_consume();
            CTG_TL_STAMP(4);
            if constexpr (TRI) {
                static_for<0, ITM>([&](auto ii) __attribute__((always_inline)) { item_mid(ii); });
                __syncthreads();
                static_for<0, ITM>([&](auto ii) __attribute__((always_inline)) { scatter_mid(ii); });
                __syncthreads();
            }
            static_for<0, IT2>([&](auto ii) __attribute__((always_inline)) {
                constexpr int I = decltype(ii)::value;
                if constexpr (RI2)
                    item2r(ri_rt0 + ri_rts * I, c_rows[I], std::integral_constant<int, I & (NSET - 1)>{},
                           std::integral_constant<int, (I > 0) ? ((I - 1) & (NSET - 1)) : -1>{}, scaled_tag);
                else
                    item2(wave + SW * I, c_rows[I], scaled_tag, std::integral_constant<bool, (I > 0)>{}, std::true_type{});
            });
            CTG_TL_STAMP(5);
            g += tile_step;
        };
        auto pass = [&](auto peel_tag) __attribute__((always_inline)) {
            static_for<0, U>([&](auto ui) __attribute__((always_inline)) {
                tile(std::integral_constant<int, (decltype(ui)::value * NT) & (GD - 1)>{},
                     std::integral_constant<bool, decltype(peel_tag)::value && decltype(ui)::value == 0>{});
            });
        };
        int64_t t = 0;
        if (my_tiles >= U) {
            pass(std::true_type{});
            for (t = U; t + U <= my_tiles; t += U) pass(std::false_type{});
        }
        if (t < my_tiles) {
            if (t == 0) tile(std::integral_constant<int, 0>{}, std::true_type{});
            else tile(std::integral_constant<int, 0>{}, std::false_type{});
        }
        drain(0, NST, std::integral_constant<int, LASTSET>{}, scaled_tag);
    } else {
        issue(regs[0], std::false_type{});
        issue(regs[1], std::false_type{});
        prep(std::false_type{});
        int slot = 0;
        for (int64_t g = tile0; g < n_tiles; g += tile_step) {
            const int64_t c_tile1 = ONE ? tile_c(g) : 0;
#pragma unroll
            for (int m = 0; m < RT1; ++m) {
                zero_acc(m);
                for (int ch = 0; ch < nch; ++ch) {
                    if (slot == 0) consume(regs[0], m, ch, std::false_type{}, std::integral_constant<int, -1>{}, scaled_tag);
                    else consume(regs[1], m, ch, std::false_type{}, std::integral_constant<int, -1>{}, scaled_tag);
                    slot ^= 1;
                }
                if constexpr (ONE) {
                    emit_one(m, c_tile1, scaled_tag);
                    drain(0, NST, std::integral_constant<int, 0>{}, scaled_tag);
                }
            }
            if constexpr (ONE) continue;
            h2_publish();
            __syncthreads();
            scatter();
            __syncthreads();
            h2_consume();
            const int64_t c_tile = tile_c(g);
            for (int item = wave; item < n_items; item += SW)
                item2(item, item_row(item, c_tile), scaled_tag, std::false_type{}, std::false_type{});
        }
    }
    };
    if (scaled) run(std::true_type{});
    else run(std::false_type{});
    if constexpr (BF3) {
        if (p.cmax != nullptr) {
            float mx = h2_vmax;
#pragma unroll
            for (int o = 32; o > 0; o >>= 1) mx = fmaxf(mx, __shfl_xor(mx, o));
            if (lane == 0 && mx > 0.f && mx < __builtin_bit_cast(float, 0x7f800000u))
                record_max(p.cmax, mx);
        }
    }
}

template <bool PACK1, bool PACK2, int RT1_, int CS1, int NCH, int IT2_, bool BR1 = false, int K2Q = 0, bool VEC = false,
          bool BF3 = false, bool RI2 = false, bool ONE = false, int ITM = 0, bool PACKM = false, bool XM = false,
          bool LM = false, bool WS = false>
__global__ __launch_bounds__(SW * 64, 1) void stem2_kernel(StemArgs p) {
    stem2_body<Bf16x3, PACK1, PACK2, RT1_, CS1, NCH, IT2_, BR1, K2Q, VEC, BF3, RI2, ONE, ITM, PACKM, XM, LM, WS>(p);
}
template <bool PACK1, bool PACK2, int RT1_, int CS1, int NCH, int IT2_, bool BR1 = false, int K2Q = 0, bool VEC = false,
          bool BF3 = false, bool RI2 = false, bool ONE = false, int ITM = 0, bool PACKM = false, bool XM = false,
          bool LM = false, bool WS = false>
__global__ __launch_bounds__(SW * 64, 1) void stem2h_kernel(StemArgs p) {
    stem2_body<Fp16x2, PACK1, PACK2, RT1_, CS1, NCH, IT2_, BR1, K2Q, VEC, BF3, RI2, ONE, ITM, PACKM, XM, LM, WS>(p);
}
template <bool PACK1, bool PACK2, int RT1_, int CS1, int NCH, int IT2_, bool BR1 = false, int K2Q = 0, bool VEC = false,
          bool BF3 = false, bool RI2 = false, bool ONE = false, int ITM = 0, bool PACKM = false, bool XM = false,
          bool LM = false, bool WS = false>
__global__ __launch_bounds__(SW * 64, 1) void stem2_kernel_p16(StemArgs p) {
    stem2_body<Bf16x3, PACK1, PACK2, RT1_, CS1, NCH, IT2_, BR1, K2Q, VEC, BF3, RI2, ONE, ITM, PACKM, XM, LM, WS, true>(p);
}
template <bool PACK1, bool PACK2, int RT1_, int CS1, int NCH, int IT2_, bool BR1 = false, int K2Q = 0, bool VEC = false,
          bool BF3 = false, bool RI2 = false, bool ONE = false, int ITM = 0, bool PACKM = false, bool XM = false,
          bool LM = false, bool WS = false>
__global__ __launch_bounds__(SW * 64, 1) void stem2h_kernel_p16(StemArgs p) {
    stem2_body<Fp16x2, PACK1, PACK2, RT1_, CS1, NCH, IT2_, BR1, K2Q, VEC, BF3, RI2, ONE, ITM, PACKM, XM, LM, WS, true>(p);
}

#ifdef CTG_STEM_TIMELINE
template <class AR>
int stem_debug_timeline(unsigned long long* out, int reset) {
    if (hipDeviceSynchronize() != hipSuccess) return -1;
    if (hipMemcpyFromSymbol(out, HIP_SYMBOL(ctg_stem_tl<AR>), sizeof(unsigned long long) * 8 * CTG_TL_TILES * 6) != hipSuccess) return -1;
    if (reset) {
        static unsigned long long z[8 * CTG_TL_TILES * 6];
        if (hipMemcpyToSymbol(HIP_SYMBOL(ctg_stem_tl<AR>), z, sizeof(z)) != hipSuccess) return -1;
    }
    return 0;
}
#endif

#ifdef CTG_STEM_BOUNDS
template <class AR>
int stem_debug_oob(unsigned long long out[2], int reset) {
    if (hipMemcpyFromSymbol(out, HIP_SYMBOL(ctg_stem_oob<AR>), 16) != hipSuccess) return -1;
    if (reset) {
        const unsigned long long z[2] = {0, 0};
        if (hipMemcpyToSymbol(HIP_SYMBOL(ctg_stem_oob<AR>), z, 16) != hipSuccess) return -1;
    }
    return 0;
}
#endif

#ifndef CTG_STEM_DEV_ONE
template <class AR, auto... A>
static auto stem_kernel() {
    if constexpr (AR::fp16) return stem2h_kernel<A...>;
    else return stem2_kernel<A...>;
}
template <class AR, auto... A>
static auto stem_kernel_p16() {
    if constexpr (AR::fp16) return stem2h_kernel_p16<A...>;
    else return stem2_kernel_p16<A...>;
}

static size_t stem2_lds_bytes(const StemArgs& p) {
    const size_t b1 = (size_t)(p.N1 == 16 ? 3 : 2) * p.N1 * (p.K1 + 4);
    const size_t b2 = (size_t)(p.N2 == 16 ? 3 : 2) * p.N2 * (p.K2 + 4);
    const size_t mid = (size_t)2 * p.rows2 * p.ld2;
    return 4 * (b1 + b2 + mid) + 8 * (size_t)p.N2;
}

static size_t stem2_lds_bytes_bf3(const StemArgs& p) {
    const size_t q1 = (size_t)(p.N1 == 16 ? 3 : 2) * p.N1 * ((p.K1 >> 4) * 48 + 8);
    const size_t q2 = (size_t)(p.N2 == 16 ? 3 : 2) * p.N2 * ((p.K2 >> 3) * 24 + 8);
    return 2 * (q1 + q2) + 4 * (size_t)2 * p.rows2 * p.ld2 + 8 * (size_t)p.N2 + 64;
}

static size_t stem2_lds_bytes_ri2(const StemArgs& p, bool b2_in_regs) {
    const size_t b1 = (size_t)(p.N1 == 16 ? 3 : 2) * p.N1 * (p.K1 + 4);
    const size_t b2 = (size_t)2 * p.N2 * (p.K2 + 4);
    const size_t mid = (size_t)3 * p.rows2 * p.ld2;
    return 4 * (b1 + (b2_in_regs ? (mid > b2 ? mid : b2) : b2 + mid)) + 8 * (size_t)p.N2;
}

static bool stem_pair16_shape(const StemArgs& p, bool ws) {
    if (!p.pair16 || p.one || p.tri || env_on("CTG_STEM_NO_PAIR16")) return false;
    const int n_rt2 = p.rows2 >> 5;
    if (p.N2 != 32 * p.ng2 || n_rt2 < 1) return false;
    if (ws) return n_rt2 == SW / 2 && p.ng2 == 2 && p.K2 == 64;
    return n_rt2 <= SW && SW % n_rt2 == 0 && n_rt2 * p.ng2 == 2 * SW;
}
#ifdef CTG_STEM_PAIR16_SYM
constexpr bool STEM_PAIR16_SYM = true;
#else
constexpr bool STEM_PAIR16_SYM = false;
#endif
static int stem_last_paired = 0;

template <class AR, bool PACK1, bool PACK2, int RT1, int CS1, int NCH, int IT2, bool BR1 = false, int K2Q = 0, bool VEC = false,
          bool BF3 = false, bool RI2 = false, bool XM = false, bool WS = false>
static hipError_t launch_stem2_t(const StemArgs& p, hipStream_t stream) {
    auto kern = stem_kernel<AR, PACK1, PACK2, RT1, CS1, NCH, IT2, BR1, K2Q, VEC, BF3, RI2, false, 0, false, XM, false, WS>();
    static unsigned long long ready = 0, ready16 = 0;
    bool paired = false;
    if constexpr (BF3 && XM && !PACK2 && NCH > 0 && ((AR::fp16 && WS && IT2 == 1) || (STEM_PAIR16_SYM && !WS && IT2 == 2))) {
        if (stem_pair16_shape(p, WS)) {
            kern = stem_kernel_p16<AR, PACK1, PACK2, RT1, CS1, NCH, IT2, BR1, K2Q, VEC, BF3, RI2, false, 0, false, XM, false, WS>();
            paired = true;
        }
    }
    stem_last_paired = paired ? 1 : 0;
    {
        const hipError_t e = lds_opt_in((const void*)kern, 160 * 1024, paired ? &ready16 : &ready);
        if (e != hipSuccess) return e;
    }
#ifdef CTG_STEM_TIMELINE
    {
        static int taken = 0;
        int on = 0, k1 = 0, n1 = 0, k2 = 0, n2 = 0;
        if (const char* v = getenv("CTG_TL_SHAPE"))
            if (sscanf(v, "%d,%d,%d,%d", &k1, &n1, &k2, &n2) == 4 && k1 == p.K1 && n1 == p.N1 && k2 == p.K2 && n2 == p.N2 && !taken)
                on = taken = 1;
        (void)hipMemcpyToSymbolAsync(HIP_SYMBOL(ctg_stem_tl_on<AR>), &on, sizeof(int), 0, hipMemcpyHostToDevice, stream);
    }
#endif
    const size_t smem = BF3 ? stem2_lds_bytes_bf3(p) : (RI2 ? stem2_lds_bytes_ri2(p, K2Q > 0) : stem2_lds_bytes(p));
    int64_t blocks = p.n_tiles < 256 ? p.n_tiles : 256;
    hipLaunchKernelGGL(kern, dim3((unsigned)blocks, 1), dim3(SW * 64), smem, stream, p);
    return hipGetLastError();
}

static size_t stem2_lds_bytes_one(const StemArgs& p, bool bf3) {
    if (bf3) return 2 * (size_t)2 * p.N1 * ((p.K1 >> 4) * 48 + 8) + 8 * (size_t)p.N1 + 64;
    return 4 * (size_t)2 * p.N1 * (p.K1 + 4) + 8 * (size_t)p.N1;
}

template <class AR, int RT1, int CS1, int NCH, bool BR1, bool VEC, bool BF3>
static hipError_t launch_stem1_t(const StemArgs& p, hipStream_t stream) {
    constexpr bool XM = BF3 && NCH > 0;
    auto kern = stem_kernel<AR, false, false, RT1, CS1, NCH, 0, BR1, 0, VEC, BF3, false, true, 0, false, XM, false, false>();
    static unsigned long long ready = 0;
    {
        const hipError_t e = lds_opt_in((const void*)kern, 160 * 1024, &ready);
        if (e != hipSuccess) return e;
    }
    int64_t blocks = p.n_tiles < 256 ? p.n_tiles : 256;
    hipLaunchKernelGGL(kern, dim3((unsigned)blocks, 1), dim3(SW * 64), stem2_lds_bytes_one(p, BF3), stream, p);
    return hipGetLastError();
}

static size_t stem3_lds_bytes(const StemArgs& p, bool bf3) {
    const size_t m1 = (size_t)p.rowsM * p.ldM, m2 = (size_t)p.rows2 * p.ld2;
    const size_t mid = 8 * (m1 > m2 ? m1 : m2);
    auto planes = [](int n) { return (size_t)(n == 16 ? 3 : 2); };
    if (bf3) {
        const size_t q = planes(p.N1) * p.N1 * ((p.K1 >> 4) * 48 + 8) + planes(p.NM) * p.NM * ((p.KM >> 3) * 24 + 8) +
                         planes(p.N2) * p.N2 * ((p.K2 >> 3) * 24 + 8);
        return 2 * q + mid + 8 * (size_t)p.N2 + 64;
    }
    const size_t b = planes(p.N1) * p.N1 * (p.K1 + 4) + planes(p.NM) * p.NM * (p.KM + 4) + planes(p.N2) * p.N2 * (p.K2 + 4);
    return 4 * b + mid + 8 * (size_t)p.N2;
}

template <bool P1, bool PM, bool P2, int RT1, int CS1, int NCH, int ITM, int IT2, bool VEC, bool BF3>
static hipError_t launch_stem3_t(const StemArgs& p, hipStream_t stream) {
    auto kern = stem2_kernel<P1, P2, RT1, CS1, NCH, IT2, (NCH <= 2), 0, VEC, BF3, false, false, ITM, PM>;
    static unsigned long long ready = 0;
    {
        const hipError_t e = lds_opt_in((const void*)kern, 160 * 1024, &ready);
        if (e != hipSuccess) return e;
    }
    int64_t blocks = p.n_tiles < 256 ? p.n_tiles : 256;
    hipLaunchKernelGGL(kern, dim3((unsigned)blocks, 1), dim3(SW * 64), stem3_lds_bytes(p, BF3), stream, p);
    return hipGetLastError();
}

#if !defined(CTG_STEM_TRIPLES_BUILD)
#define CTG_STEM_TRI(X)
#elif defined(CTG_STEM_TRI_DEV)
#define CTG_STEM_TRI(X) \
    X(true, true, true, 2, 1, 1, 2, 2, false) X(false, false, false, 1, 1, 2, 1, 1, false) \
    X(true, false, true, 2, 1, 1, 1, 1, false) X(true, false, false, 1, 1, 1, 1, 1, true)
#else
#define CTG_STEM_TRI(X) \
    X(true, true, false, 2, 1, 1, 2, 1, true) X(true, true, false, 2, 1, 1, 2, 1, false) \
    X(true, false, true, 2, 1, 1, 1, 2, false) X(false, true, true, 1, 1, 2, 2, 2, false) \
    X(false, true, false, 1, 2, 1, 2, 2, false) X(false, false, true, 1, 1, 2, 1, 2, false) \
    X(false, false, true, 1, 1, 4, 1, 1, true) \
    X(true, false, true, 2, 1, 1, 1, 1, false) X(true, false, true, 2, 1, 1, 1, 1, true) \
    X(false, true, true, 1, 4, 2, 2, 2, true) X(false, false, false, 1, 1, 2, 1, 4, false) \
    X(true, false, false, 1, 1, 1, 1, 1, true)
#endif

static bool stem3_instantiated(bool p1, bool pm, bool p2, int rt1, int cs1, int nch, int itm, int it2, bool vec) {
#define CTG_STEM_HAS3(A, M, B, R, CS, NC, IM, IT, V) \
    if (p1 == A && pm == M && p2 == B && rt1 == R && cs1 == CS && nch == NC && itm == IM && it2 == IT && vec == V) return true;
    CTG_STEM_TRI(CTG_STEM_HAS3)
#undef CTG_STEM_HAS3
    return false;
}

struct Stem3Shape { bool p1, pm, p2; int rt1, cs1, nch, itm, it2; bool vec; };
static Stem3Shape stem3_shape(const StemArgs& p) {
    Stem3Shape s;
    s.p1 = p.N1 == 16; s.pm = p.NM == 16; s.p2 = p.N2 == 16;
    s.cs1 = p.N1 >= 32 ? p.N1 / 32 : 1;
    s.rt1 = ((1 << (p.nr1 - 5)) * s.cs1) / SW;
    s.nch = p.K1 / 16;
    const int im = (p.rowsM / 32) * p.ngM, i2 = (p.rows2 / 32) * p.ng2;
    s.itm = im % SW == 0 ? im / SW : 0;
    s.it2 = i2 % SW == 0 ? i2 / SW : 0;
    s.vec = p.vec != 0;
    return s;
}

static bool stem3_supported_shape(const StemArgs& p) {
    auto k_ok = [](int k) { return k == 16 || k == 32 || k == 64 || k == 128; };
    auto n_ok = [](int n) { return n == 16 || n == 32 || n == 64 || n == 128; };
    if (!p.tri || p.one || !k_ok(p.K1) || !k_ok(p.KM) || !k_ok(p.K2) || !n_ok(p.N1) || !n_ok(p.NM) || !n_ok(p.N2)) return false;
    const int cs1 = p.N1 >= 32 ? p.N1 / 32 : 1;
    if (p.nr1 < 5 || p.nr1 > 9) return false;
    const int units = (1 << (p.nr1 - 5)) * cs1;
    if (units != 8 && units != 16) return false;
    if (p.rowsM < 32 || (p.rowsM & 31) || p.ldM != p.KM + 4 || p.rows2 < 32 || (p.rows2 & 31) || p.ld2 != p.K2 + 4) return false;
    if ((int64_t)(1 << p.nr1) * p.N1 != (int64_t)p.rowsM * p.KM || (int64_t)p.rowsM * p.NM != (int64_t)p.rows2 * p.K2) return false;
    if (p.ngM != (p.NM >= 32 ? p.NM / 32 : 1) || p.ng2 != (p.N2 >= 32 ? p.N2 / 32 : 1)) return false;
    const Stem3Shape s = stem3_shape(p);
    if (s.itm < 1 || s.itm > 2 || s.it2 < 1 || s.it2 > 4) return false;
    if (!stem3_instantiated(s.p1, s.pm, s.p2, s.rt1, s.cs1, s.nch, s.itm, s.it2, s.vec)) return false;
// ... 137 lines not shown
    if (s.p1 == P1 && s.p2 == P2 && s.rt1 == R && s.cs1 == CS && s.nch == NC && s.it2 == IT && s.br1 == B1 && \
        s.k2q == KQ && s.vec == V && s.ri2 == RI)                                                      \
        return 1;
    CTG_STEM_INST(CTG_STEM_HAS)
#undef CTG_STEM_HAS
    return 0;
}

static bool stem2_has_geo(const StemShape& s) {
    if (env_on("CTG_STEM_GENERIC") || s.it2 == 0) return false;
#define CTG_STEM_HASG(P1, P2, R, CS, NC, IT, V)                                                         \
    if (s.p1 == P1 && s.p2 == P2 && s.rt1 == R && s.cs1 == CS && s.nch == NC && s.it2 == IT && s.vec == V) return true;
    CTG_STEM_GEO(CTG_STEM_HASG)
#undef CTG_STEM_HASG
    return false;
}

static bool stem_wants_16bit(const StemArgs& p) {
    const int v = env_state("CTG_STEM_BF16X3");
    return v >= 0 ? v == 1 : p.bf3 != 0;
}

static bool stem2_bf3(const StemArgs& p) {
    const bool want = stem_wants_16bit(p);
    if (p.one) return want && stem1_static(stem2_shape(p, true)) && stem2_lds_bytes_one(p, true) <= 160 * 1024;
    return want && stem2_has_geo(stem2_shape(p, true)) && (p.K2 & 7) == 0 && stem2_lds_bytes_bf3(p) <= 160 * 1024;
}

template <class AR>
static int stem2_bf3_form(const StemArgs& p) {
    int form = AR::max_form;
    if (const char* v = getenv("CTG_STEM_FORM")) form = atoi(v) < form ? atoi(v) : form;
    if (form < 1 || form == 2) form = 1;
    const int items = (p.rows2 / 32) * p.ng2, units = (1 << (p.nr1 - 5)) * (p.N1 >= 32 ? p.N1 / 32 : 1);
    if (form == 3 && !(items <= 2 * SW && (p.N1 == 16 || units == SW))) form = 1;
    if (form == 3 && items == 2 * SW && p.N2 >= 32) form = 1;
    if (items >= 4 * SW) form = 0;
    return form;
}

template <class AR>
static void stem_kernel_name(const StemArgs& p, char* buf, size_t n) {
    const StemShape s = stem2_shape(p);
    const char* const kn = AR::kernel_name;
    auto tf = [](bool b) { return b ? "true" : "false"; };
    if (p.tri) {
        const Stem3Shape t = stem3_shape(p);
        snprintf(buf, n, "%s<%s,%s,%d,%d,%d,%d,%s,0,%s,%s,false,false,%d,%s>", kn, tf(t.p1), tf(t.p2), t.rt1, t.cs1,
                 t.nch, t.it2, tf(t.nch <= BR1_CHUNKS), tf(t.vec), tf(stem_wants_16bit(p)), t.itm, tf(t.pm));
        return;
    }
    if (p.one) {
        const bool st = stem1_static(s), b3 = stem2_bf3(p);
        if (st && b3)
            snprintf(buf, n, "%s<false,false,%d,%d,%d,0,%s,0,%s,true,false,true,0,false,true,false>", kn, s.rt1, s.cs1,
                     s.nch, tf(s.nch <= BR1_CHUNKS), tf(s.vec));
        else
            snprintf(buf, n, "%s<false,false,%d,%d,%d,0,%s,0,%s,%s,false,true>", kn, s.rt1, s.cs1, st ? s.nch : 0,
                     tf(st && (b3 ? s.nch <= BR1_CHUNKS : p.K1 <= 64)), tf(s.vec), tf(b3));
        return;
    }
    if (stem2_bf3(p)) {
        const int form = stem2_bf3_form<AR>(p);
        if (form == 0)
            snprintf(buf, n, "%s<%s,%s,%d,%d,%d,%d,%s,0,%s,true,false,false>", kn, tf(s.p1), tf(s.p2), s.rt1, s.cs1,
                     s.nch, s.it2, tf(s.nch <= BR1_CHUNKS), tf(s.vec));
        else
            snprintf(buf, n, "%s<%s,%s,%d,%d,%d,%d,%s,0,%s,true,false,false,0,false,true,false,%s>", kn, tf(s.p1), tf(s.p2),
                     s.rt1, s.cs1, s.nch, s.it2, tf(form >= 3 ? stem_br1_ws(s.cs1, s.nch) : s.nch <= BR1_CHUNKS), tf(s.vec),
                     tf(form >= 3));
    }
    else if (stem2_variant(p))
        snprintf(buf, n, "%s<%s,%s,%d,%d,%d,%d,%s,%d,%s,false,%s,false>", kn, tf(s.p1), tf(s.p2), s.rt1, s.cs1, s.nch,
                 s.it2, tf(s.br1), s.k2q, tf(s.vec), tf(s.ri2));
    else
        snprintf(buf, n, "%s<%s,%s,%d,%d,0,0,false,0,%s,false,false,false>", kn, tf(s.p1), tf(s.p2), s.rt1, s.cs1,
                 tf(s.vec));
}

static bool stem_uses_16bit(const StemArgs& p) { return !p.tri && stem2_supported_shape(p) && stem2_bf3(p); }

template <class AR>
static hipError_t launch_stem(const StemArgs& p, hipStream_t stream) {
    if (!stem2_supported_shape(p)) return hipErrorInvalidValue;
    if constexpr (AR::fp16) {
        if (!stem_uses_16bit(p)) return hipErrorInvalidValue;
    } else {
        if (p.tri) {
            const Stem3Shape t = stem3_shape(p);
            const bool b3 = stem_wants_16bit(p);
#define CTG_STEM_GO3T(A, M, B, R, CS, NC, IM, IT, V)                                                                  \
    if (t.p1 == A && t.pm == M && t.p2 == B && t.rt1 == R && t.cs1 == CS && t.nch == NC && t.itm == IM && t.it2 == IT && \
        t.vec == V)                                                                                                   \
        return b3 ? launch_stem3_t<A, M, B, R, CS, NC, IM, IT, V, true>(p, stream)                                    \
                  : launch_stem3_t<A, M, B, R, CS, NC, IM, IT, V, false>(p, stream);
            CTG_STEM_TRI(CTG_STEM_GO3T)
#undef CTG_STEM_GO3T
            return hipErrorInvalidValue;
        }
    }
    if (p.one) {
        const StemShape s = stem2_shape(p, true);
        const bool b3 = stem2_bf3(p);
        if (stem1_static(s)) {
#define CTG_STEM_GO1(R, CS, NC, V)                                                                            \
    if (s.rt1 == R && s.cs1 == CS && s.nch == NC && s.vec == V) {                                             \
        if (b3) return launch_stem1_t<AR, R, CS, NC, (NC <= BR1_CHUNKS), V, true>(p, stream);                 \
        if constexpr (!AR::fp16) return launch_stem1_t<AR, R, CS, NC, (NC <= 4), V, false>(p, stream);        \
    }
            CTG_STEM_ONE(CTG_STEM_GO1)
#undef CTG_STEM_GO1
        }
        if constexpr (!AR::fp16) {
#define CTG_STEM_CASE1(R, CS)                                                               \
    if (s.rt1 == R && s.cs1 == CS)                                                          \
        return s.vec ? launch_stem1_t<AR, R, CS, 0, false, true, false>(p, stream)          \
                     : launch_stem1_t<AR, R, CS, 0, false, false, false>(p, stream);
            CTG_STEM_CASE1(1, 1) CTG_STEM_CASE1(2, 1) CTG_STEM_CASE1(1, 2) CTG_STEM_CASE1(2, 2)
            CTG_STEM_CASE1(1, 4) CTG_STEM_CASE1(2, 4)
#undef CTG_STEM_CASE1
        }
        return hipErrorInvalidValue;
    }
    if (stem2_bf3(p)) {
        const StemShape s = stem2_shape(p, true);
        const int form = stem2_bf3_form<AR>(p);
#define CTG_STEM_GO3(P1, P2, R, CS, NC, IT, V)                                                                           \
    if (s.p1 == P1 && s.p2 == P2 && s.rt1 == R && s.cs1 == CS && s.nch == NC && s.it2 == IT && s.vec == V) {             \
        if constexpr (AR::max_form >= 3 && IT <= 2 && (P1 || R == 1) && (P2 || IT < 2)) {                                \
            if (form == 3)                                                                                               \
                return launch_stem2_t<AR, P1, P2, R, CS, NC, IT, stem_br1_ws(CS, NC), 0, V, true, false, true, true>(p, stream);  \
        }                                                                                                                \
        if constexpr (IT < 4) {                                                                                          \
            if (form == 1)                                                                                               \
                return launch_stem2_t<AR, P1, P2, R, CS, NC, IT, (NC <= BR1_CHUNKS), 0, V, true, false, true, false>(p, stream); \
        } else {                                                                                                         \
            if (form == 0) return launch_stem2_t<AR, P1, P2, R, CS, NC, IT, (NC <= BR1_CHUNKS), 0, V, true>(p, stream);  \
        }                                                                                                                \
        return hipErrorInvalidValue;                                                                                     \
    }
        CTG_STEM_GEO(CTG_STEM_GO3)
#undef CTG_STEM_GO3
    }
    if constexpr (!AR::fp16) {
        const StemShape s = stem2_shape(p);
        if (stem2_variant(p)) {
#define CTG_STEM_GO(P1, P2, R, CS, NC, IT, B1, KQ, V, RI)                                              \
    if (s.p1 == P1 && s.p2 == P2 && s.rt1 == R && s.cs1 == CS && s.nch == NC && s.it2 == IT && s.br1 == B1 && \
        s.k2q == KQ && s.vec == V && s.ri2 == RI)                                                      \
        return launch_stem2_t<AR, P1, P2, R, CS, NC, IT, B1, KQ, V, false, RI>(p, stream);
            CTG_STEM_INST(CTG_STEM_GO)
#undef CTG_STEM_GO
        }
#define CTG_STEM_CASE(P1, P2, R, CS)                                                                    \
    if (s.p1 == P1 && s.p2 == P2 && s.rt1 == R && s.cs1 == CS)                                          \
        return s.vec ? launch_stem2_t<AR, P1, P2, R, CS, 0, 0, false, 0, true>(p, stream)               \
                     : launch_stem2_t<AR, P1, P2, R, CS, 0, 0, false, 0, false>(p, stream);
#define CTG_STEM_CASES(P2)             \
    CTG_STEM_CASE(true, P2, 1, 1)      \
    CTG_STEM_CASE(true, P2, 2, 1)      \
    CTG_STEM_CASE(false, P2, 1, 1)     \
    CTG_STEM_CASE(false, P2, 2, 1)     \
    CTG_STEM_CASE(false, P2, 1, 2)     \
    CTG_STEM_CASE(false, P2, 2, 2)     \
    CTG_STEM_CASE(false, P2, 1, 4)     \
    CTG_STEM_CASE(false, P2, 2, 4)
// ... 11 lines not shown
```

cotengra_amd/runtime.py:

```python

from __future__ import annotations

import ctypes as C
import os

import numpy as np

_LIB_PATH = os.environ.get("CTG_LIB") or os.path.join(os.path.dirname(os.path.abspath(__file__)), "lib", "libctg_hip.so")
ABI_VERSION = 10

SYMBOLS = (
    "ctg_abi_version",
    "ctg_last_error",
    "ctg_plan_create",
    "ctg_plan_destroy",
    "ctg_plan_nslices",
    "ctg_plan_workspace_bytes",
    "ctg_exec_create",
    "ctg_exec_destroy",
    "ctg_exec_set_stream",
    "ctg_exec_upload_inputs_host",
    "ctg_exec_upload_inputs_device",
    "ctg_exec_zero_result",
    "ctg_exec_set_strip_exponent",
    "ctg_exec_set_stem_arithmetic",
    "ctg_exec_get_exponent",
    "ctg_exec_run_slices",
    "ctg_exec_run_slice_list",
    "ctg_plan_share_units",
    "ctg_plan_share_slice_ids",
    "ctg_exec_run_share",
    "ctg_exec_slice_batch",
    "ctg_exec_device_bytes",
    "ctg_stem_triple_instantiated",
    "ctg_exec_launch_count",
    "ctg_exec_profile_slice",
    "ctg_exec_step_kernel",
    "ctg_exec_lds_form",
    "ctg_exec_step_paired_stores",
    "ctg_exec_step_stem_max",
    "ctg_plan_stem_pair16",
    "ctg_exec_sync",
    "ctg_exec_result_ptr",
    "ctg_exec_result_stats",
    "ctg_exec_sample_result",
    "ctg_exec_sample_info",
    "ctg_exec_range_audit",
    "ctg_exec_result_topk",
    "ctg_exec_result_marginal",
    "ctg_exec_result_rdm",
    "ctg_exec_result_pauli",
    "ctg_exec_result_pauli_apply",
    "ctg_exec_download_result",
    "ctg_exec_download_arena",
    "ctg_exec_get_state",
    "ctg_exec_set_state",
    "ctg_exec_state_dtype",
    "ctg_exec_get_state_wide",
    "ctg_exec_set_state_wide",
    "ctg_comm_get_unique_id",
    "ctg_comm_init",
    "ctg_comm_info",
    "ctg_comm_destroy",
    "ctg_exec_reduce",
    "ctg_path_greedy",
    "ctg_slice_greedy",
    "ctg_subtree_reconfigure",
    "ctg_subtree_reconfigure_timed",
)


class CtgError(RuntimeError):
    """A call into libctg_hip.so failed."""


class CommError(CtgError):
    """RCCL is missing or a collective failed (CTG_E_COMM)."""


class PlanDesc(C.Structure):

    _fields_ = [
        ("dtype", C.c_int32),
        ("n_inputs", C.c_int64),
        ("input_sizes", C.POINTER(C.c_int64)),
        ("input_offsets", C.POINTER(C.c_int64)),
        ("inputs_elems", C.c_int64),
        ("arena_elems", C.c_int64),
        ("result_elems", C.c_int64),
        ("n_steps", C.c_int64),
        ("steps", C.POINTER(C.c_int64)),
        ("n_table_words", C.c_int64),
        ("tables", C.POINTER(C.c_int64)),
        ("n_sliced", C.c_int64),
        ("slice_sizes", C.POINTER(C.c_int64)),
        ("slice_fixed", C.POINTER(C.c_int64)),
        ("slice_strides", C.POINTER(C.c_int64)),
        ("slice_group", C.POINTER(C.c_int64)),
    ]


_lib = None


def lib_path():
    return _LIB_PATH


def load():
    global _lib
    if _lib is not None:
        return _lib
    if not os.path.exists(_LIB_PATH):
        raise ImportError(
            f"{_LIB_PATH} not found: build the HIP extension first "
            "(python -c 'import __graft_entry__ as g; g.build()'). "
            "cotengra_amd has no CPU fallback."
        )
    try:
        import torch
    except ImportError:
        pass
    lib = C.CDLL(_LIB_PATH)
    i64p = C.POINTER(C.c_int64)
    vp = C.c_void_p
    lib.ctg_abi_version.restype = C.c_int
    lib.ctg_last_error.restype = C.c_char_p
    protos = {
        "ctg_plan_create": [C.POINTER(PlanDesc), C.POINTER(vp)],
        "ctg_plan_destroy": [vp],
        "ctg_plan_nslices": [vp, i64p],
        "ctg_plan_workspace_bytes": [vp, i64p],
        "ctg_exec_create": [vp, C.c_int, vp, vp, C.POINTER(vp)],
        "ctg_exec_destroy": [vp],
        "ctg_exec_set_stream": [vp, vp],
        "ctg_exec_upload_inputs_host": [vp, C.POINTER(vp)],
        "ctg_exec_upload_inputs_device": [vp, C.POINTER(vp)],
        "ctg_exec_zero_result": [vp],
        "ctg_exec_set_strip_exponent": [vp, C.c_int, C.c_int],
        "ctg_exec_set_stem_arithmetic": [vp, C.c_int],
        "ctg_exec_get_exponent": [vp, C.POINTER(C.c_double), C.POINTER(C.c_int)],
        "ctg_exec_run_slices": [vp, C.c_int64, C.c_int64, C.c_int64],
        "ctg_exec_run_slice_list": [vp, i64p, C.c_int64],
        "ctg_plan_share_units": [vp, C.c_int64, C.c_int64, i64p, i64p],
        "ctg_plan_share_slice_ids": [vp, C.c_int64, C.c_int64, C.c_int64, C.c_int64, i64p],
        "ctg_exec_run_share": [vp, C.c_int64, C.c_int64, C.c_int64, C.c_int64],
        "ctg_exec_slice_batch": [vp, i64p],
        "ctg_exec_device_bytes": [vp, i64p],
        "ctg_stem_triple_instantiated": [C.c_int] * 9,
        "ctg_exec_launch_count": [vp, i64p, i64p],
        "ctg_exec_profile_slice": [vp, C.c_int64, C.POINTER(C.c_float)],
        "ctg_exec_step_kernel": [vp, C.c_int64, C.c_char_p, C.c_int64],
        "ctg_exec_lds_form": [vp, C.c_int64, C.c_int64, i64p, C.c_char_p, C.c_int64],
        "ctg_exec_step_paired_stores": [vp, C.c_int64, C.POINTER(C.c_int)],
        "ctg_exec_step_stem_max": [vp, C.c_int64, C.c_int64, C.POINTER(C.c_float)],
        "ctg_plan_stem_pair16": [vp, C.c_int64, C.POINTER(C.c_int)],
        "ctg_exec_sync": [vp],
        "ctg_exec_result_ptr": [vp, C.POINTER(vp)],
        "ctg_exec_result_stats": [vp, C.POINTER(C.c_double), C.POINTER(C.c_double), C.POINTER(C.c_double), i64p],
        "ctg_exec_sample_result": [vp, C.POINTER(C.c_double), C.c_int64, i64p, vp, C.POINTER(C.c_double)],
        "ctg_exec_sample_info": [vp, C.POINTER(C.c_double), C.POINTER(C.c_double), C.POINTER(C.c_double), i64p,
                                 C.POINTER(C.c_float)],
        "ctg_exec_range_audit": [vp, C.c_int64, i64p, C.POINTER(C.c_double)],
        "ctg_exec_result_topk": [vp, C.c_int64, i64p, vp, C.POINTER(C.c_double)],
        "ctg_exec_result_marginal": [vp, C.c_int64, i64p, C.POINTER(C.c_int32), C.POINTER(C.c_double)],
        "ctg_exec_result_rdm": [vp, C.c_int64, i64p, C.POINTER(C.c_int32), vp],
        "ctg_exec_result_pauli": [vp, C.c_int64, i64p, C.c_int64, C.POINTER(C.c_uint8), C.POINTER(C.c_double)],
        "ctg_exec_result_pauli_apply": [vp, C.c_int64, i64p, C.c_int64, C.POINTER(C.c_uint8), C.POINTER(C.c_double), vp, vp],
        "ctg_exec_download_result": [vp, vp],
        "ctg_exec_download_arena": [vp, C.c_int64, C.c_int64, vp],
        "ctg_exec_get_state": [vp, vp, C.POINTER(C.c_double), C.POINTER(C.c_int)],
        "ctg_exec_set_state": [vp, vp, C.c_double, C.c_int],
        "ctg_exec_state_dtype": [vp, C.POINTER(C.c_int)],
        "ctg_exec_get_state_wide": [vp, vp, C.POINTER(C.c_double), C.POINTER(C.c_int)],
        "ctg_exec_set_state_wide": [vp, vp, C.c_double, C.c_int],
        "ctg_comm_get_unique_id": [vp],
        "ctg_comm_init": [vp, C.c_int, C.c_int, C.c_int, C.POINTER(vp)],
        "ctg_comm_info": [vp, C.POINTER(C.c_int), C.POINTER(C.c_int), C.POINTER(C.c_int)],
        "ctg_comm_destroy": [vp],
        "ctg_exec_reduce": [vp, vp, C.c_int],
        "ctg_path_greedy": [C.c_int64, i64p, i64p, C.c_int64, i64p, C.c_int64, C.POINTER(C.c_double),
                            C.c_double, C.c_double, C.c_int64, C.c_uint64, i64p],
        "ctg_slice_greedy": [C.c_int64, i64p, i64p, C.c_int64, i64p, C.c_int64, C.POINTER(C.c_double),
                             i64p, C.c_double, C.c_int, C.c_int64, i64p, i64p],
        "ctg_subtree_reconfigure": [C.c_int64, i64p, i64p, C.c_int64, i64p, C.c_int64, C.POINTER(C.c_double),
                                    i64p, C.c_int64, C.c_int64, C.c_double, i64p],
        "ctg_subtree_reconfigure_timed": [C.c_int64, i64p, i64p, C.c_int64, i64p, C.c_int64,
                                          C.POINTER(C.c_double), i64p, C.c_int64, C.c_int64,
                                          C.POINTER(C.c_double), C.c_int64, C.c_double, i64p],
    }
    for name, argtypes in protos.items():
        fn = getattr(lib, name)
        fn.argtypes = argtypes
        fn.restype = C.c_int
    if lib.ctg_abi_version() != ABI_VERSION:
        raise ImportError(
            f"libctg_hip.so ABI {lib.ctg_abi_version()} != expected {ABI_VERSION}; rebuild."
        )
    _lib = lib
    return lib


def _check(rc):
    if rc != 0:
        msg = load().ctg_last_error().decode("utf-8", "replace")
        if rc in (-1, -6):
            raise ValueError(msg)
        if rc == -3:
            raise MemoryError(msg)
        if rc == -5:
            raise CommError(msg)
        raise CtgError(f"[{rc}] {msg}")


def _i64p(arr):
    return arr.ctypes.data_as(C.POINTER(C.c_int64))


def check_topk_k(k):
    import operator

    if isinstance(k, (bool, np.bool_)):
        raise TypeError(f"k = {k!r} is not an integer.")
    try:
        k = operator.index(k)
    except TypeError:
        raise TypeError(f"k = {k!r} is not an integer.") from None
    if k < 1:
        raise ValueError(f"k = {k}: need at least 1.")
    return k


def rdm_dim(extents, keep):
    d = 1
    for n, f in zip(extents, keep):
        if n < 1:
            raise ValueError(f"extent {n} is not positive.")
# ... 228 lines not shown

    STEM_ARITHMETICS = {"fp32": 0, "bf16x3": 1, "fp16x2": 2}

    def set_stem_arithmetic(self, mode):
        if mode is True:
            mode = 1
        elif mode is False:
            mode = 0
        elif isinstance(mode, str):
            mode = self.STEM_ARITHMETICS[mode]
        _check(load().ctg_exec_set_stem_arithmetic(self.handle, int(mode)))

    def get_exponent(self):
        e, z = C.c_double(), C.c_int()
        _check(load().ctg_exec_get_exponent(self.handle, C.byref(e), C.byref(z)))
        return e.value, bool(z.value)

    def run_slice_list(self, ids):
        arr = np.ascontiguousarray(ids, dtype=np.int64)
        _check(load().ctg_exec_run_slice_list(self.handle, arr.ctypes.data_as(C.POINTER(C.c_int64)), arr.size))

    def run_share(self, rank=0, world=1, unit_first=0, unit_count=-1):
        _check(load().ctg_exec_run_share(self.handle, int(rank), int(world), int(unit_first), int(unit_count)))

    def run_slices(self, first=0, count=None, stride=1):
        if count is None:
            count = (self.plan.nslices - first + stride - 1) // stride
        _check(load().ctg_exec_run_slices(self.handle, first, count, stride))

    @property
    def batch(self):
        n = C.c_int64()
        _check(load().ctg_exec_slice_batch(self.handle, C.byref(n)))
        return n.value

    def device_bytes(self):
        n = C.c_int64()
        _check(load().ctg_exec_device_bytes(self.handle, C.byref(n)))
        return n.value

    def launch_count(self):
        ns, nl = C.c_int64(), C.c_int64()
        _check(load().ctg_exec_launch_count(self.handle, C.byref(ns), C.byref(nl)))
        return ns.value, nl.value

    def profile_slice(self, slice_id=0):
        ms = (C.c_float * max(len(self.plan.steps), 1))()
        _check(load().ctg_exec_profile_slice(self.handle, slice_id, ms))
        return np.asarray(ms[: len(self.plan.steps)], dtype=np.float64)

    def step_kernels(self):
        buf = C.create_string_buffer(160)
        names = []
        for s in range(len(self.plan.steps)):
            _check(load().ctg_exec_step_kernel(self.handle, s, buf, 160))
            names.append(buf.value.decode())
        return names

    def lds_forms(self):
        fn = load().ctg_exec_lds_form
        buf = C.create_string_buffer(96)
        main = C.c_int64()
        out = []
        while True:
            recs = []
            while True:
                _check(fn(self.handle, len(out), len(recs), C.byref(main), buf, 96))
                if main.value < 0:
                    break
                recs.append((buf.value.decode(), int(main.value)))
            if not recs:
                return out
            out.append(recs)

    def step_paired_stores(self):
        fn = load().ctg_exec_step_paired_stores
        out = []
        for s in range(len(self.plan.steps)):
            v = C.c_int()
            _check(fn(self.handle, s, C.byref(v)))
            out.append(bool(v.value))
        return out

    def step_stem_max(self, step, z=0):
        v = C.c_float()
        _check(load().ctg_exec_step_stem_max(self.handle, int(step), int(z), C.byref(v)))
        return float(v.value)

    def sync(self):
        _check(load().ctg_exec_sync(self.handle))

    def result_ptr(self):
        p = C.c_void_p()
        _check(load().ctg_exec_result_ptr(self.handle, C.byref(p)))
        return p.value

    def download_result(self):
        out = np.empty(self.plan.result_shape, dtype=np.dtype(self.plan.dtype))
        _check(load().ctg_exec_download_result(self.handle, C.c_void_p(out.ctypes.data)))
        return out


    def result_stats(self):
        s, q, m, i = C.c_double(), C.c_double(), C.c_double(), C.c_int64()
        _check(load().ctg_exec_result_stats(self.handle, C.byref(s), C.byref(q), C.byref(m), C.byref(i)))
        return s.value, q.value, m.value, i.value

    def sample_result(self, uniforms):
        u = np.ascontiguousarray(uniforms, dtype=np.float64).reshape(-1)
        n = u.size
        idx = np.empty(n, dtype=np.int64)
        elems = np.empty(n, dtype=np.dtype(self.plan.dtype))
        p = np.empty(n, dtype=np.float64)
        dp = C.POINTER(C.c_double)
        _check(load().ctg_exec_sample_result(self.handle, u.ctypes.data_as(dp), n, _i64p(idx),
                                             C.c_void_p(elems.ctypes.data), p.ctypes.data_as(dp)))
        return idx, elems, p

    def sample_info(self):
        s, q, m, i = C.c_double(), C.c_double(), C.c_double(), C.c_int64()
        ms = (C.c_float * 2)()
        _check(load().ctg_exec_sample_info(self.handle, C.byref(s), C.byref(q), C.byref(m), C.byref(i), ms))
        return s.value, q.value, m.value, i.value, (ms[0], ms[1])


    TOPK_MAX = 1 << 20

    def topk_result(self, k):
        k = check_topk_k(k)
        idx = np.empty(k, dtype=np.int64)
        elems = np.empty(k, dtype=np.dtype(self.plan.dtype))
        p = np.empty(k, dtype=np.float64)
        _check(load().ctg_exec_result_topk(self.handle, k, _i64p(idx), C.c_void_p(elems.ctypes.data),
                                           p.ctypes.data_as(C.POINTER(C.c_double))))
        return idx, elems, p

    def marginal_result(self, extents, keep):
        ext = np.ascontiguousarray(extents, dtype=np.int64).reshape(-1)
        kp = np.ascontiguousarray(keep, dtype=np.int32).reshape(-1)
        if ext.size != kp.size:
            raise ValueError(f"{ext.size} extents and {kp.size} keep entries.")
        m = 1
        for d, f in zip(ext.tolist(), kp.tolist()):
            if d < 1:
                raise ValueError(f"extent {d} is not positive.")
            if f == 1:
                m *= d
        out = np.empty(m, dtype=np.float64)
        _check(load().ctg_exec_result_marginal(self.handle, ext.size, _i64p(ext), kp.ctypes.data_as(C.POINTER(C.c_int32)),
                                               out.ctypes.data_as(C.POINTER(C.c_double))))
        return out


    RDM_MAX_DIM = 64

    def rdm_result(self, extents, keep):
        ext = np.ascontiguousarray(extents, dtype=np.int64).reshape(-1)
        kp = np.ascontiguousarray(keep, dtype=np.int32).reshape(-1)
        if ext.size != kp.size:
            raise ValueError(f"{ext.size} extents and {kp.size} keep entries.")
        d = rdm_dim(ext.tolist(), kp.tolist())
        cplx = np.dtype(self.plan.dtype).kind == "c"
        out = np.empty((d, d), dtype=np.complex128 if cplx else np.float64)
        _check(load().ctg_exec_result_rdm(self.handle, ext.size, _i64p(ext), kp.ctypes.data_as(C.POINTER(C.c_int32)),
                                          C.c_void_p(out.ctypes.data)))
        return out
# ... 141 lines not shown
```

include/ctg_hip.h:

```cpp
#ifndef CTG_HIP_H
#define CTG_HIP_H

#include <stdint.h>

#ifdef __cplusplus
extern "C" {
#endif

#define CTG_ABI_VERSION 10

enum { CTG_F32 = 0, CTG_F64 = 1, CTG_C64 = 2, CTG_C128 = 3 };

enum {
    CTG_OK = 0,
    CTG_E_INVALID = -1,
    CTG_E_HIP = -2,
    CTG_E_NOMEM = -3,
    CTG_E_BOUNDS = -4,
    CTG_E_COMM = -5,
    CTG_E_NORM = -6
};

#define CTG_STEP_WORDS 48

typedef struct ctg_plan_desc {
    int32_t dtype;
    int64_t n_inputs;
    const int64_t* input_sizes;
    const int64_t* input_offsets;
    int64_t inputs_elems;
    int64_t arena_elems;
    int64_t result_elems;
    int64_t n_steps;
    const int64_t* steps;
    int64_t n_table_words;
    const int64_t* tables;
    int64_t n_sliced;
    const int64_t* slice_sizes;
    const int64_t* slice_fixed;
    const int64_t* slice_strides;
    const int64_t* slice_group;
} ctg_plan_desc;

typedef struct ctg_plan ctg_plan;
typedef struct ctg_exec ctg_exec;
typedef struct ctg_comm ctg_comm;

int ctg_abi_version(void);
const char* ctg_last_error(void);

int ctg_plan_create(const ctg_plan_desc* desc, ctg_plan** out);
int ctg_plan_destroy(ctg_plan* plan);
int ctg_plan_nslices(const ctg_plan* plan, int64_t* nslices);
int ctg_plan_workspace_bytes(const ctg_plan* plan, int64_t bytes[4]);

int ctg_exec_create(const ctg_plan* plan, int device, void* stream,
                    void* ext_result, ctg_exec** out);
int ctg_exec_destroy(ctg_exec* exec);
int ctg_exec_set_stream(ctg_exec* exec, void* stream);

int ctg_exec_upload_inputs_host(ctg_exec* exec, const void* const* ptrs);
int ctg_exec_upload_inputs_device(ctg_exec* exec, const void* const* ptrs);

int ctg_exec_zero_result(ctg_exec* exec);

int ctg_exec_set_strip_exponent(ctg_exec* exec, int strip_exponent, int check_zero);

int ctg_exec_set_stem_arithmetic(ctg_exec* exec, int mode);
int ctg_exec_get_exponent(ctg_exec* exec, double* exponent, int* zero);

int ctg_exec_run_slices(ctg_exec* exec, int64_t first, int64_t count, int64_t stride);

int ctg_exec_slice_batch(ctg_exec* exec, int64_t* batch);
int ctg_exec_run_slice_list(ctg_exec* exec, const int64_t* ids, int64_t n);
int ctg_plan_share_units(const ctg_plan* plan, int64_t rank, int64_t world, int64_t* units, int64_t* slices_per_unit);
int ctg_plan_share_slice_ids(const ctg_plan* plan, int64_t rank, int64_t world, int64_t unit_first,
                             int64_t unit_count, int64_t* ids);
int ctg_exec_run_share(ctg_exec* exec, int64_t rank, int64_t world, int64_t unit_first, int64_t unit_count);
int ctg_exec_device_bytes(ctg_exec* exec, int64_t* bytes);
int ctg_stem_triple_instantiated(int p1, int pm, int p2, int rt1, int cs1, int nch, int itm, int it2, int vec);

int ctg_exec_launch_count(ctg_exec* exec, int64_t* steps, int64_t* launches);

int ctg_exec_profile_slice(ctg_exec* exec, int64_t slice_id, float* ms);

int ctg_exec_step_kernel(ctg_exec* exec, int64_t step, char* buf, int64_t buflen);
int ctg_exec_lds_form(ctg_exec* exec, int64_t comp, int64_t rec, int64_t* main_step, char* buf, int64_t buflen);
int ctg_exec_step_paired_stores(ctg_exec* exec, int64_t step, int* paired);
int ctg_exec_step_stem_max(ctg_exec* exec, int64_t step, int64_t z, float* mx);
int ctg_plan_stem_pair16(ctg_plan* plan, int64_t step, int* ok);

int ctg_exec_sync(ctg_exec* exec);
int ctg_exec_result_ptr(ctg_exec* exec, void** dev_ptr);
int ctg_exec_download_result(ctg_exec* exec, void* host_out);
int ctg_exec_result_stats(ctg_exec* exec, double* sum_p, double* sum_p2, double* max_p, int64_t* argmax);
int ctg_exec_sample_result(ctg_exec* exec, const double* u, int64_t n, int64_t* idx, void* elems, double* p);
int ctg_exec_sample_info(ctg_exec* exec, double* sum_p, double* sum_p2, double* max_p, int64_t* argmax, float* pass_ms);
#define CTG_RANGE_WORDS 260
int ctg_exec_range_audit(ctg_exec* exec, int64_t slice_id, int64_t* rows, double* sumsq);
#define CTG_TOPK_MAX (1 << 20)
int ctg_exec_result_topk(ctg_exec* exec, int64_t k, int64_t* idx, void* elems, double* p);
#define CTG_MARGINAL_PARTIALS (1 << 22)
int ctg_exec_result_marginal(ctg_exec* exec, int64_t rank, const int64_t* extents, const int32_t* keep, double* out);
#define CTG_RDM_MAX_DIM 64
int ctg_exec_result_rdm(ctg_exec* exec, int64_t rank, const int64_t* extents, const int32_t* keep, void* out);
#define CTG_PAULI_MAX_STRINGS 4096
int ctg_exec_result_pauli(ctg_exec* exec, int64_t rank, const int64_t* extents, int64_t m, const uint8_t* ops, double* out);
int ctg_exec_result_pauli_apply(ctg_exec* exec, int64_t rank, const int64_t* extents, int64_t m, const uint8_t* ops,
                                const double* coeffs, void* dev_out, void* host_out);
int ctg_exec_download_arena(ctg_exec* exec, int64_t offset, int64_t n, void* host_out);

int ctg_exec_get_state(ctg_exec* exec, void* host_result, double* exponent, int* zero);
int ctg_exec_set_state(ctg_exec* exec, const void* host_result, double exponent, int zero);
int ctg_exec_state_dtype(ctg_exec* exec, int* dtype);
int ctg_exec_get_state_wide(ctg_exec* exec, void* host_sum, double* exponent, int* zero);
int ctg_exec_set_state_wide(ctg_exec* exec, const void* host_sum, double exponent, int zero);

#define CTG_UNIQUE_ID_BYTES 128
int ctg_comm_get_unique_id(void* id_out );
int ctg_comm_init(const void* id, int rank, int world, int device, ctg_comm** out);
int ctg_comm_info(const ctg_comm* comm, int* rank, int* world, int* device);
int ctg_comm_destroy(ctg_comm* comm);
int ctg_exec_reduce(ctg_exec* exec, ctg_comm* comm, int root);


int ctg_path_greedy(int64_t n_inputs, const int64_t* offsets, const int64_t* inds, int64_t n_out,
                    const int64_t* out_inds, int64_t n_inds, const double* sizes, double costmod,
                    double temperature, int64_t max_neighbors, uint64_t seed, int64_t* ssa_path);

int ctg_slice_greedy(int64_t n_inputs, const int64_t* offsets, const int64_t* inds, int64_t n_out,
                     const int64_t* out_inds, int64_t n_inds, const double* sizes,
                     const int64_t* ssa_path, double target_log2_size, int allow_outer,
                     int64_t max_sliced, int64_t* sliced, int64_t* n_sliced);

int ctg_subtree_reconfigure(int64_t n_inputs, const int64_t* offsets, const int64_t* inds, int64_t n_out,
                            const int64_t* out_inds, int64_t n_inds, const double* sizes,
                            const int64_t* ssa_path_in, int64_t subtree_size, int64_t maxiter,
                            double write_factor, int64_t* ssa_path_out);

int ctg_subtree_reconfigure_timed(int64_t n_inputs, const int64_t* offsets, const int64_t* inds,
                                  int64_t n_out, const int64_t* out_inds, int64_t n_inds,
                                  const double* sizes, const int64_t* ssa_path_in, int64_t subtree_size,
                                  int64_t maxiter, const double* mac_rate_by_log2k, int64_t n_rates,
                                  double elem_rate, int64_t* ssa_path_out);

#ifdef __cplusplus
}
#endif
#endif
```

Measured before the change: 175100 billion FLOP/s.

## Add shared-rows stem kernel variant so each wave covers two column groups

Adds a shared-rows (SR) variant of the single-step 16-bit stem kernel. Each wave now computes two 32-column groups of the same row tile, so the A fragments are loaded once and reused across both column groups. Two tiles are packed per block, with waves split between them. The variant is enabled by default for the RT1=1, CS1=4 geometry and can be disabled with an env variable; it also adds a query API reporting which steps used it. It trades a higher register load (two accumulator sets per wave) for less A-fragment traffic and issue overhead.

```diff
diff --git a/cotengra_amd/csrc/ctg_common.h b/cotengra_amd/csrc/ctg_common.h
--- a/cotengra_amd/csrc/ctg_common.h
+++ b/cotengra_amd/csrc/ctg_common.h
@@ -459,6 +459,8 @@
 void stem2h_kernel_name(const StemArgs& p, char* buf, size_t n);
 int stem2_last_paired();
 int stem2h_last_paired();
+int stem2_last_shared_rows();
+int stem2h_last_shared_rows();
 
 hipError_t launch_single(int dtype, const StepArgs& p, hipStream_t stream);
 bool pair_bf16x3_on(const StepArgs& p);
diff --git a/cotengra_amd/csrc/ctg_exec_state.h b/cotengra_amd/csrc/ctg_exec_state.h
--- a/cotengra_amd/csrc/ctg_exec_state.h
+++ b/cotengra_amd/csrc/ctg_exec_state.h
@@ -58,6 +58,7 @@
     int64_t plan_steps = 0;
     std::vector<char> rec_wanted;
     std::vector<char> wave_member;
+    std::vector<char> stem_shared_ran;
     std::vector<char> stem_paired_ran;
     std::vector<char> stem_h2_ran;
     std::vector<ctg::MfmaHints> hints;
diff --git a/cotengra_amd/csrc/ctg_runtime.hip b/cotengra_amd/csrc/ctg_runtime.hip
--- a/cotengra_amd/csrc/ctg_runtime.hip
+++ b/cotengra_amd/csrc/ctg_runtime.hip
@@ -1152,6 +1152,7 @@
                 }
                 if (err == hipSuccess) err = h2 ? launch_stem2h(q, stream) : launch_stem2(q, stream);
                 if (err == hipSuccess) e->stem_paired_ran[s] = (char)(h2 ? stem2h_last_paired() : stem2_last_paired());
+                if (err == hipSuccess) e->stem_shared_ran[s] = (char)(h2 ? stem2h_last_shared_rows() : stem2_last_shared_rows());
             }
             break;
         }
@@ -1847,6 +1848,7 @@
             }
             e->stem_h2_ran.assign(p->n_steps, 0);
             e->stem_paired_ran.assign(p->n_steps, 0);
+            e->stem_shared_ran.assign(p->n_steps, 0);
             if (e->wave_member.size() != (size_t)p->n_steps) e->wave_member.assign(p->n_steps, 0);
             (void)stems;
             if (p->dtype == CTG_C64) {
@@ -2461,6 +2463,13 @@
     return CTG_OK;
 }
 
+int ctg_exec_step_shared_rows(ctg_exec* e, int64_t step, int* shared) {
+    if (!e || !shared) return fail(CTG_E_INVALID, "null argument");
+    if (step < 0 || step >= e->plan->n_steps) return fail(CTG_E_INVALID, "step out of range");
+    *shared = (size_t)step < e->stem_shared_ran.size() && e->stem_shared_ran[step] ? 1 : 0;
+    return CTG_OK;
+}
+
 int ctg_exec_step_stem_max(ctg_exec* e, int64_t step, int64_t z, float* mx) {
     if (!e || !mx) return fail(CTG_E_INVALID, "null argument");
     const ctg_plan* p = e->plan;
diff --git a/cotengra_amd/csrc/ctg_stem.hip b/cotengra_amd/csrc/ctg_stem.hip
--- a/cotengra_amd/csrc/ctg_stem.hip
+++ b/cotengra_amd/csrc/ctg_stem.hip
@@ -2,13 +2,16 @@
 
 namespace ctg {
 #ifdef CTG_STEM_DEV_ONE
-#ifdef CTG_STEM_DEV_P16
+#if defined(CTG_STEM_DEV_SR)
+template __global__ void stem2_kernel_sr<CTG_STEM_DEV_ONE>(StemArgs);
+#elif defined(CTG_STEM_DEV_P16)
 template __global__ void stem2_kernel_p16<CTG_STEM_DEV_ONE>(StemArgs);
 #else
 template __global__ void stem2_kernel<CTG_STEM_DEV_ONE>(StemArgs);
 #endif
 #else
 int stem2_last_paired() { return stem_last_paired; }
+int stem2_last_shared_rows() { return stem_last_shared; }
 bool stem2_supported(const StemArgs& p) { return stem2_supported_shape(p); }
 bool stem3_supported(const StemArgs& p) { return stem3_supported_shape(p); }
 bool stem2_uses_bf3(const StemArgs& p) { return stem_uses_16bit(p); }
diff --git a/cotengra_amd/csrc/ctg_stem_h2.hip b/cotengra_amd/csrc/ctg_stem_h2.hip
--- a/cotengra_amd/csrc/ctg_stem_h2.hip
+++ b/cotengra_amd/csrc/ctg_stem_h2.hip
@@ -2,13 +2,16 @@
 
 namespace ctg {
 #ifdef CTG_STEM_DEV_ONE
-#ifdef CTG_STEM_DEV_P16
+#if defined(CTG_STEM_DEV_SR)
+template __global__ void stem2h_kernel_sr<CTG_STEM_DEV_ONE>(StemArgs);
+#elif defined(CTG_STEM_DEV_P16)
 template __global__ void stem2h_kernel_p16<CTG_STEM_DEV_ONE>(StemArgs);
 #else
 template __global__ void stem2h_kernel<CTG_STEM_DEV_ONE>(StemArgs);
 #endif
 #else
 int stem2h_last_paired() { return stem_last_paired; }
+int stem2h_last_shared_rows() { return stem_last_shared; }
 bool stem2h_supported(const StemArgs& p) { return stem2_supported_shape(p); }
 bool stem2h_uses_h2(const StemArgs& p) { return stem_uses_16bit(p); }
 void stem2h_kernel_name(const StemArgs& p, char* buf, size_t n) { stem_kernel_name<Fp16x2>(p, buf, n); }
diff --git a/cotengra_amd/csrc/ctg_stem_impl.h b/cotengra_amd/csrc/ctg_stem_impl.h
--- a/cotengra_amd/csrc/ctg_stem_impl.h
+++ b/cotengra_amd/csrc/ctg_stem_impl.h
@@ -241,9 +241,11 @@
 constexpr bool STEM_NT_STORES = CTG_STEM_NT_STORES != 0;
 constexpr bool STEM_GATHER_PORTIONS = CTG_STEM_GATHER_PORTIONS != 0;
 template <class AR, bool PACK1, bool PACK2, int RT1_, int CS1, int NCH, int IT2_, bool BR1, int K2Q, bool VEC, bool BF3,
-          bool RI2, bool ONE, int ITM, bool PACKM, bool XM, bool LM, bool WS, bool P16 = false>
+          bool RI2, bool ONE, int ITM, bool PACKM, bool XM, bool LM, bool WS, bool P16 = false, bool SR = false>
 __device__ __forceinline__ void stem2_body(const StemArgs& p) {
     constexpr bool TRI = ITM > 0;
+    static_assert(!SR || (ONE && XM && RT1_ == 1 && CS1 >= 2 && !BR1 && !P16),
+                  "shared rows: a static 16-bit single step with column groups, B1's fragments from LDS");
     static_assert(!P16 || (XM && !PACK2 && NCH > 0 && ((WS && IT2_ == 1) || (!WS && IT2_ == 2))),
                   "paired stores: a wave whose two items are the two column groups of a row tile");
     static_assert(!LM, "reserved (the limb intermediate was removed): kernel names stay 17 arguments long");
@@ -251,7 +253,8 @@
     static_assert(!AR::fp16 || !TRI, "fp16 x 2: pairs and single steps");
     static_assert(!WS || (XM && !ONE && IT2_ > 0 && IT2_ <= 2 && (PACK1 || RT1_ == 1)), "specialised waves: a static 16-bit pair");
     constexpr int PW = WS ? 4 : SW;
-    constexpr int RT1 = WS ? 2 * RT1_ : RT1_;
+    constexpr int SRG = 2;
+    constexpr int RT1 = SR ? SRG : (WS ? 2 * RT1_ : RT1_);
     constexpr int IT2 = WS ? 2 * IT2_ : IT2_;
     static_assert(!XM || (BF3 && !TRI && NCH > 0), "two-accumulator real part: bf16 x 3, static, no three-step tile");
     constexpr bool XM1 = XM && !PACK1 && !WS;
@@ -263,9 +266,11 @@
     static_assert(K2Q == 0 || PACK2 || IT2 == 1 || RI2, "B2 in registers: one column group per wave");
     static_assert(!RI2 || (!PACK2 && !BF3 && NCH > 0 && IT2 > 0), "row-interleaved step 2: fp32, >= 32 columns, static");
     constexpr bool SH1 = WS && CS1 > 1 && RT1 % CS1 == 0;
-    constexpr int CG1 = SH1 ? CS1 : 1;
+    constexpr int CG1 = SR ? SRG : (SH1 ? CS1 : 1);
     constexpr int RR1 = RT1 / CG1;
     constexpr int RTW = SH1 ? PW : PW / CS1;
+    constexpr int SRW = SW / SRG;
+    constexpr int SRS = CS1 / SRG > 0 ? CS1 / SRG : 1;
     constexpr bool STATIC = NCH > 0;
     extern __shared__ __attribute__((aligned(16))) char smem[];
     const int K1 = p.K1, N1 = p.N1, K2 = K2Q > 0 ? 4 * K2Q : p.K2, N2 = p.N2;
@@ -303,8 +308,9 @@
     const int l31 = lane & 31;
     const bool producer = !WS || wave < PW;
     const int wave1 = WS ? (wave & (PW - 1)) : wave;
-    const int wrt = SH1 ? wave1 : wave1 / CS1;
-    const int wcol = SH1 ? 0 : (wave1 % CS1) * 32;
+    const int wrt = SR ? (wave1 % SRW) / SRS : (SH1 ? wave1 : wave1 / CS1);
+    const int wcol = SR ? ((wave1 % SRW) % SRS) * 32 * SRG
+                        : (SH1 ? 0 : (wave1 % CS1) * 32);
 
     const int64_t z = (int64_t)p.z0 + blockIdx.y;
     const c64* __restrict__ A = (const c64*)p.A + (sload64(p.soffA + z * p.zsA) + z * p.zA);
@@ -411,7 +417,9 @@
         mid_rt[m] = ONE ? 0 : __builtin_amdgcn_readfirstlane(ri_off((int)sload64(p.mid_row + 32 * (wrt + RTW * (m / CG1)))));
         one_rt[m] = ONE ? sload64(p.out_row + 32 * (wrt + RTW * (m / CG1))) : 0;
     }
-    const int64_t one_col = ONE ? p.out_col[wcol + l31] : 0;
+    int64_t one_col[CG1];
+#pragma unroll
+    for (int cg = 0; cg < CG1; ++cg) one_col[cg] = ONE ? p.out_col[wcol + 32 * cg + l31] : 0;
     auto mid_t = [&](int t) __attribute__((always_inline)) {
         return ((t & 1) ? mid_o[0] : 0) + ((t & 2) ? mid_o[1] : 0) + ((t & 4) ? mid_o[2] : 0) + ((t & 8) ? mid_o[3] : 0);
     };
@@ -536,8 +544,9 @@
     const int n_rt2 = p.rows2 >> 5;
     const int n_items = n_rt2 * p.ng2;
     const int64_t n_tiles = p.n_tiles;
-    const int64_t tile0 = blockIdx.x, tile_step = gridDim.x;
-    const int64_t my_tiles = (n_tiles - tile0 + tile_step - 1) / tile_step;
+    const int64_t tile0 = SR ? (int64_t)SRG * blockIdx.x + wave1 / SRW : blockIdx.x;
+    const int64_t tile_step = SR ? (int64_t)SRG * gridDim.x : gridDim.x;
+    const int64_t my_tiles = (SR && tile0 >= n_tiles) ? 0 : (n_tiles - tile0 + tile_step - 1) / tile_step;
     const int64_t last_tile = tile0 + (my_tiles - 1) * tile_step;
 
     constexpr int GD = WS ? CTG_STEM_WS_DEPTH : ((NCH > 0 && CTG_STEM_DEPTH == 4 && ((RT1 * NCH) & 1) == 0) ? 4 : 2);
@@ -675,6 +684,20 @@
             }
         }
     };
+    auto emit_one = [&](int m, int64_t c_tile, auto scaled_tag) __attribute__((always_inline)) {
+        constexpr bool SC = decltype(scaled_tag)::value;
+#pragma unroll
+        for (int t = 0; t < 16; ++t) {
+            float2 v;
+            const float xr = XM1 ? ax[m][t] - axm[m][t] : ax[m][t];
+            v.x = SC ? xr * alpha * alpha2 : xr;
+            v.y = SC ? ay[m][t] * alpha * alpha2 : ay[m][t];
+            if constexpr (BF3) h2_vmax = fmaxf(h2_vmax, fmaxf(fabsf(v.x), fabsf(v.y)));
+            pv[RI2 ? 0 : t] = v;
+        }
+        pdst = C + 2 * (c_tile + one_rt[m] + out_lane + one_col[m % CG1]);
+    };
+    int64_t sr_ctile = 0;
     auto consume = [&](c64 (&r)[8], int m, int ch, auto always_tag, auto drain_tag, auto scaled_tag)
                        __attribute__((always_inline)) {
         constexpr bool DRAIN = decltype(drain_tag)::value >= 0;
@@ -695,11 +718,12 @@
 #pragma unroll
                 for (int q = 0; q < 4; ++q) fire2(r, q, base, always_tag);
             }
+            constexpr bool LAZYB = SR && AR::limbs == 3;
 #pragma unroll
             for (int q = 0; q < 3; ++q) {
                 if (!PACK1 && !XM1) n3[q] = __builtin_bit_cast(bf16x8, __builtin_bit_cast(u32x4, i3[q]) ^ 0x80008000u);
 #pragma unroll
-                for (int cg = 0; cg < CG1; ++cg) {
+                for (int cg = 0; cg < (LAZYB ? 1 : CG1); ++cg) {
                     if constexpr (BR1) {
                         bp3[cg][q] = b1r3[cg][ch][q][0];
                         bq3[cg][q] = b1r3[cg][ch][q][1];
@@ -714,6 +738,56 @@
             f32x16 zero16;
 #pragma unroll
             for (int u = 0; u < 16; ++u) zero16[u] = 0.f;
+            if constexpr (SR) {
+                auto refill = [&](int t) __attribute__((always_inline)) {
+                    if constexpr (GP) {
+                        constexpr int P = AR::products;
+                        const int i = AR::t_index(t);
+#pragma unroll
+                        for (int q = (4 * i + P - 1) / P; q < (4 * (i + 1) + P - 1) / P; ++q) fire2(r, q, base, always_tag);
+                    }
+                };
+                auto prod = [&](int cg, int t) __attribute__((always_inline)) {
+                    const int ta = bf3_ta(t), tb = bf3_tb(t);
+                    ax[cg] = AR::mfma(r3[ta], bp3[cg][tb], (fresh && t == 0) ? zero16 : ax[cg]);
+                    ay[cg] = AR::mfma(r3[ta], bq3[cg][tb], (fresh && t == 0) ? zero16 : ay[cg]);
+                    axm[cg] = AR::mfma(i3[ta], bq3[cg][tb], (fresh && t == 0) ? zero16 : axm[cg]);
+                    ay[cg] = AR::mfma(i3[ta], bp3[cg][tb], ay[cg]);
+                };
+                if (LAZYB || ch == 0) {
+#pragma unroll
+                    for (int cg = 0; cg < CG1; ++cg) {
+                        if constexpr (DRAIN) emit_one(cg, sr_ctile, scaled_tag);
+#pragma unroll
+                        for (int t = 0; t < 6; t += AR::t_step(t)) {
+                            if (cg == 0) refill(t);
+                            if (LAZYB && cg + 1 < CG1 && t + AR::t_step(t) >= 6) {
+#pragma unroll
+                                for (int q = 0; q < 3; ++q) {
+                                    bp3[cg + 1][q] = *(const bf16x8*)(q1p + (cg + 1) * q1cg + ch * 48 + q * 8);
+                                    bq3[cg + 1][q] = *(const bf16x8*)(q1q + (cg + 1) * q1cg + ch * 48 + q * 8);
+                                }
+                            }
+                            prod(cg, t);
+                            __builtin_amdgcn_sched_barrier(0);
+                            if constexpr (DRAIN)
+                                drain(AR::t_index(t) * NST / AR::products, (AR::t_index(t) + 1) * NST / AR::products, drain_tag, scaled_tag);
+                        }
+                    }
+                } else {
+#pragma unroll
+                    for (int t = 0; t < 6; t += AR::t_step(t)) {
+                        refill(t);
+#pragma unroll
+                        for (int cg = 0; cg < CG1; ++cg) prod(cg, t);
+                        __builtin_amdgcn_sched_barrier(0);
+                    }
+                }
+                __builtin_amdgcn_sched_barrier(0);
+                prep(always_tag);
+                __builtin_amdgcn_sched_barrier(0);
+                return;
+            }
 #pragma unroll
             for (int t = 0; t < 6; t += AR::t_step(t)) {
                 const int ta = bf3_ta(t), tb = bf3_tb(t);
@@ -1201,19 +1275,6 @@
             dst[m2_t(t)] = mx[I][t];
             if (!PACKM) dst[PLANE + m2_t(t)] = my[I][t];
         }
-    };
-    auto emit_one = [&](int m, int64_t c_tile, auto scaled_tag) __attribute__((always_inline)) {
-        constexpr bool SC = decltype(scaled_tag)::value;
-#pragma unroll
-        for (int t = 0; t < 16; ++t) {
-            float2 v;
-            const float xr = XM1 ? ax[m][t] - axm[m][t] : ax[m][t];
-            v.x = SC ? xr * alpha * alpha2 : xr;
-            v.y = SC ? ay[m][t] * alpha * alpha2 : ay[m][t];
-            if constexpr (BF3) h2_vmax = fmaxf(h2_vmax, fmaxf(fabsf(v.x), fabsf(v.y)));
-            pv[RI2 ? 0 : t] = v;
-        }
-        pdst = C + 2 * (c_tile + one_rt[m] + out_lane + one_col);
     };
     int h2_par = 0;
     auto h2_publish = [&]() __attribute__((always_inline)) {
@@ -1315,16 +1376,30 @@
             drain(0, NST, std::integral_constant<int, 0>{}, scaled_tag);
         }
     } else if constexpr (STATIC) {
-        constexpr int NT = RT1 * NCH;
+        constexpr int NT = RR1 * NCH;
         constexpr int U = (NT % GD) ? 2 : 1;
         static_assert((U * NT) % GD == 0, "a pass of U tiles returns to gather set 0");
         constexpr int LASTSET = RI2 ? ((IT2 > 0 ? IT2 - 1 : 0) & (NSET - 1)) : 0;
+        if constexpr (SR) {
+            if (my_tiles == 0) return;
+        }
         static_for<0, GD>([&](auto gi) __attribute__((always_inline)) { issue(regs[decltype(gi)::value], std::true_type{}); });
         prep(std::true_type{});
         int64_t g = tile0;
         auto tile = [&](auto slot0_tag, auto first_tag) __attribute__((always_inline)) {
             constexpr int SLOT0 = decltype(slot0_tag)::value;
             constexpr bool FIRST = decltype(first_tag)::value;
+            if constexpr (SR) {
+                const int64_t c_tile = tile_c(g);
+                static_for<0, NCH>([&](auto ci) __attribute__((always_inline)) {
+                    constexpr int CH = decltype(ci)::value;
+                    consume(regs[(SLOT0 + CH) & (GD - 1)], 0, CH, std::true_type{},
+                            std::integral_constant<int, (CH == 0 && !FIRST) ? 0 : -1>{}, scaled_tag);
+                });
+                sr_ctile = c_tile;
+                g += tile_step;
+                return;
+            }
             if constexpr (ONE) {
                 const int64_t c_tile = tile_c(g);
                 static_for<0, RT1>([&](auto mi) __attribute__((always_inline)) {
@@ -1403,7 +1478,14 @@
             if (t == 0) tile(std::integral_constant<int, 0>{}, std::true_type{});
             else tile(std::integral_constant<int, 0>{}, std::false_type{});
         }
-        drain(0, NST, std::integral_constant<int, LASTSET>{}, scaled_tag);
+        if constexpr (SR) {
+            static_for<0, CG1>([&](auto ci) __attribute__((always_inline)) {
+                emit_one(decltype(ci)::value, sr_ctile, scaled_tag);
+                drain(0, NST, std::integral_constant<int, 0>{}, scaled_tag);
+            });
+        } else {
+            drain(0, NST, std::integral_constant<int, LASTSET>{}, scaled_tag);
+        }
     } else {
         issue(regs[0], std::false_type{});
         issue(regs[1], std::false_type{});
@@ -1474,6 +1556,19 @@
     stem2_body<Fp16x2, PACK1, PACK2, RT1_, CS1, NCH, IT2_, BR1, K2Q, VEC, BF3, RI2, ONE, ITM, PACKM, XM, LM, WS, true>(p);
 }
 
+template <bool PACK1, bool PACK2, int RT1_, int CS1, int NCH, int IT2_, bool BR1 = false, int K2Q = 0, bool VEC = false,
+          bool BF3 = false, bool RI2 = false, bool ONE = false, int ITM = 0, bool PACKM = false, bool XM = false,
+          bool LM = false, bool WS = false>
+__global__ __launch_bounds__(SW * 64, 1) void stem2_kernel_sr(StemArgs p) {
+    stem2_body<Bf16x3, PACK1, PACK2, RT1_, CS1, NCH, IT2_, BR1, K2Q, VEC, BF3, RI2, ONE, ITM, PACKM, XM, LM, WS, false, true>(p);
+}
+template <bool PACK1, bool PACK2, int RT1_, int CS1, int NCH, int IT2_, bool BR1 = false, int K2Q = 0, bool VEC = false,
+          bool BF3 = false, bool RI2 = false, bool ONE = false, int ITM = 0, bool PACKM = false, bool XM = false,
+          bool LM = false, bool WS = false>
+__global__ __launch_bounds__(SW * 64, 1) void stem2h_kernel_sr(StemArgs p) {
+    stem2_body<Fp16x2, PACK1, PACK2, RT1_, CS1, NCH, IT2_, BR1, K2Q, VEC, BF3, RI2, ONE, ITM, PACKM, XM, LM, WS, false, true>(p);
+}
+
 #ifdef CTG_STEM_TIMELINE
 template <class AR>
 int stem_debug_timeline(unsigned long long* out, int reset) {
@@ -1509,6 +1604,11 @@
 static auto stem_kernel_p16() {
     if constexpr (AR::fp16) return stem2h_kernel_p16<A...>;
     else return stem2_kernel_p16<A...>;
+}
+template <class AR, auto... A>
+static auto stem_kernel_sr() {
+    if constexpr (AR::fp16) return stem2h_kernel_sr<A...>;
+    else return stem2_kernel_sr<A...>;
 }
 
 static size_t stem2_lds_bytes(const StemArgs& p) {
@@ -1583,16 +1683,30 @@
     return 4 * (size_t)2 * p.N1 * (p.K1 + 4) + 8 * (size_t)p.N1;
 }
 
+constexpr bool stem_shared_rows_geo(int rt1, int cs1, int nch, bool br1, bool bf3) {
+    return bf3 && rt1 == 1 && cs1 == 4 && nch > 0 && nch < 8 && !br1;
+}
+static int stem_last_shared = 0;
+
 template <class AR, int RT1, int CS1, int NCH, bool BR1, bool VEC, bool BF3>
 static hipError_t launch_stem1_t(const StemArgs& p, hipStream_t stream) {
     constexpr bool XM = BF3 && NCH > 0;
     auto kern = stem_kernel<AR, false, false, RT1, CS1, NCH, 0, BR1, 0, VEC, BF3, false, true, 0, false, XM, false, false>();
-    static unsigned long long ready = 0;
+    static unsigned long long ready = 0, ready_sr = 0;
+    bool shared = false;
+    if constexpr (stem_shared_rows_geo(RT1, CS1, NCH, BR1, BF3)) {
+        if (!env_on("CTG_STEM_NO_SHARED_ROWS")) {
+            kern = stem_kernel_sr<AR, false, false, RT1, CS1, NCH, 0, BR1, 0, VEC, BF3, false, true, 0, false, XM, false, false>();
+            shared = true;
+        }
+    }
+    stem_last_shared = shared ? 1 : 0;
     {
-        const hipError_t e = lds_opt_in((const void*)kern, 160 * 1024, &ready);
+        const hipError_t e = lds_opt_in((const void*)kern, 160 * 1024, shared ? &ready_sr : &ready);
         if (e != hipSuccess) return e;
     }
-    int64_t blocks = p.n_tiles < 256 ? p.n_tiles : 256;
+    const int64_t groups = shared ? (p.n_tiles + 1) / 2 : p.n_tiles;
+    int64_t blocks = groups < 256 ? groups : 256;
     hipLaunchKernelGGL(kern, dim3((unsigned)blocks, 1), dim3(SW * 64), stem2_lds_bytes_one(p, BF3), stream, p);
     return hipGetLastError();
 }
@@ -1896,6 +2010,7 @@
 
 template <class AR>
 static hipError_t launch_stem(const StemArgs& p, hipStream_t stream) {
+    stem_last_shared = 0;
     if (!stem2_supported_shape(p)) return hipErrorInvalidValue;
     if constexpr (AR::fp16) {
         if (!stem_uses_16bit(p)) return hipErrorInvalidValue;
diff --git a/cotengra_amd/runtime.py b/cotengra_amd/runtime.py
--- a/cotengra_amd/runtime.py
+++ b/cotengra_amd/runtime.py
@@ -38,6 +38,7 @@
     "ctg_exec_step_kernel",
     "ctg_exec_lds_form",
     "ctg_exec_step_paired_stores",
+    "ctg_exec_step_shared_rows",
     "ctg_exec_step_stem_max",
     "ctg_plan_stem_pair16",
     "ctg_exec_sync",
@@ -153,6 +154,7 @@
         "ctg_exec_step_kernel": [vp, C.c_int64, C.c_char_p, C.c_int64],
         "ctg_exec_lds_form": [vp, C.c_int64, C.c_int64, i64p, C.c_char_p, C.c_int64],
         "ctg_exec_step_paired_stores": [vp, C.c_int64, C.POINTER(C.c_int)],
+        "ctg_exec_step_shared_rows": [vp, C.c_int64, C.POINTER(C.c_int)],
         "ctg_exec_step_stem_max": [vp, C.c_int64, C.c_int64, C.POINTER(C.c_float)],
         "ctg_plan_stem_pair16": [vp, C.c_int64, C.POINTER(C.c_int)],
         "ctg_exec_sync": [vp],
@@ -547,6 +549,15 @@
             out.append(bool(v.value))
         return out
 
+    def step_shared_rows(self):
+        fn = load().ctg_exec_step_shared_rows
+        out = []
+        for s in range(len(self.plan.steps)):
+            v = C.c_int()
+            _check(fn(self.handle, s, C.byref(v)))
+            out.append(bool(v.value))
+        return out
+
     def step_stem_max(self, step, z=0):
         v = C.c_float()
         _check(load().ctg_exec_step_stem_max(self.handle, int(step), int(z), C.byref(v)))
diff --git a/include/ctg_hip.h b/include/ctg_hip.h
--- a/include/ctg_hip.h
+++ b/include/ctg_hip.h
@@ -87,6 +87,7 @@
 int ctg_exec_step_kernel(ctg_exec* exec, int64_t step, char* buf, int64_t buflen);
 int ctg_exec_lds_form(ctg_exec* exec, int64_t comp, int64_t rec, int64_t* main_step, char* buf, int64_t buflen);
 int ctg_exec_step_paired_stores(ctg_exec* exec, int64_t step, int* paired);
+int ctg_exec_step_shared_rows(ctg_exec* exec, int64_t step, int* shared);
 int ctg_exec_step_stem_max(ctg_exec* exec, int64_t step, int64_t z, float* mx);
 int ctg_plan_stem_pair16(ctg_plan* plan, int64_t step, int* ok);
 
```

New measurement: 175700 billion FLOP/s, median of 4. Within noise of the previous version (+0.3%).
